# JGCRI/xanthos

Hardware: AMD Instinct MI355X
Metric: cell-months/sec (pm_abcd_mrtm, 67,420 cells) (higher is better)
Workload: dtype f64

## Files before the change

### include/xanthos_hip.h

```cpp
#ifndef XANTHOS_HIP_H
#define XANTHOS_HIP_H

#include <stddef.h>
#include <stdint.h>

#ifdef __cplusplus
extern "C" {
#endif

#define XH_OK 0
#define XH_ERR_ARG 1
#define XH_ERR_HIP 2
#define XH_ERR_LIMIT 3
#define XH_ERR_DEVICE 4

#define XH_MAX_LCS 32

typedef struct xh_ctx xh_ctx;
typedef struct xh_route_plan xh_route_plan;

int xh_abi_version(void);
int xh_device_count(int *n);
int xh_ctx_create(int device, xh_ctx **out);
void xh_ctx_destroy(xh_ctx *ctx);
// ... 39 lines not shown
int xh_timing_reset(xh_ctx *ctx);
int xh_mark_begin(xh_ctx *ctx, const char *name);
int xh_mark_end(xh_ctx *ctx);
int xh_timing_enable(xh_ctx *ctx, int on);
int xh_timing_get(xh_ctx *ctx, const char *name, double *total_ms, int64_t *launches);

typedef struct xh_pm_tables {
    int32_t nlcs;
    const double *cL, *beta, *rslimit, *Tminopen, *Tminclose, *VPDclose, *VPDopen, *RBLmin, *RBLmax, *rc,
        *emiss;
    const double *alpha, *lai, *laimin, *laimax;
} xh_pm_tables;

int xh_pm_pet(xh_ctx *ctx, const xh_pm_tables *h_tab,
              int64_t ncell, int32_t nmonths,
              int32_t start_year,
              int32_t n_lc_years, const int32_t *h_lc_years,
              int32_t water_idx, int32_t snow_idx,
              const double *d_tas, const double *d_tmin, const double *d_rhs, const double *d_wind,
              const double *d_rsds, const double *d_rlds,
              const double *d_tairprev,
              const double *d_lct,
              const double *d_elev,
              double *d_pet);

int xh_abcd(xh_ctx *ctx, int64_t ncell, int32_t nmonths, int32_t spinup, int32_t n_groups,
            const int32_t *h_basin_index, const int32_t *h_par_index, int64_t npar_rows, const double *d_pars,
            const double *d_pet, const double *d_precip, const double *d_tmin,
            double *d_aet, double *d_q, double *d_sav,
            double *d_sm0, double *d_gw0);

int xh_hargreaves_pet(xh_ctx *ctx, int64_t ncell, int32_t nmonths,
                      const double *d_temp, const double *d_dtr,
                      const double *d_lat_rad,
                      const double *h_solar_dec, const double *h_dr, const double *h_ndays,
                      double *d_pet);

int xh_hs_pet(xh_ctx *ctx, int64_t ncell, int32_t nmonths,
              const double *d_tas, const double *d_tmax, const double *d_tmin,
              const double *d_lat_deg,
              const double *h_ndays,
              double *d_pet);

#define XH_DAYLIGHT_REFERENCE 0
#define XH_DAYLIGHT_MONTHLY 1
int xh_thornthwaite_pet(xh_ctx *ctx, int64_t ncell, int32_t nmonths, int32_t start_year, int32_t daylight_mode,
                        const double *d_tas,
                        const double *d_lat_rad,
                        double *d_pet,
                        double *d_daylight);

int xh_gwam(xh_ctx *ctx, int64_t ncell, int32_t nmonths, int32_t spinup, int32_t precip_col_spinup,
            int32_t precip_col_sim, double indexing,
            const double *d_pet, const double *d_precip,
            const double *d_sm_max, const double *d_sm0,
            double *d_aet, double *d_q, double *d_sav,
            double *d_sm_end);

int xh_route_plan_create(xh_ctx *ctx, int64_t ncell, const int64_t *h_indptr, const int32_t *h_indices,
                         const int8_t *h_sign, xh_route_plan **out);
void xh_route_plan_destroy(xh_route_plan *plan);
int xh_route_plan_info(const xh_route_plan *plan, int64_t info[16]);

int xh_route_plan_prepare(xh_ctx *ctx, xh_route_plan *plan, const double *h_flow_dist, const double *h_velocity, double dt);

int xh_route_plan_stats(xh_route_plan *plan, int64_t max_words, uint64_t *h_words, int64_t *n_words);

int xh_mrtm_downstream(int64_t ncell, int32_t nrow, int32_t ncol, const int64_t *h_id, const int32_t *h_ilon,
                       const int32_t *h_ilat, const double *h_flowdir, int64_t *h_dsid);
int xh_mrtm_upstream(int64_t ncell, int32_t nrow, int32_t ncol, const int64_t *h_id, const int32_t *h_ilon,
                     const int32_t *h_ilat, const int64_t *h_dsid, int64_t *h_upid);
int xh_mrtm_um_csr(int64_t ncell, const int64_t *h_upid, int64_t *h_indptr, int32_t *h_indices, int8_t *h_sign);

#define XH_ROUTE_DEFAULT 0
#define XH_ROUTE_FORCE_FALLBACK 1
#define XH_ROUTE_ATOMIC 2
#define XH_ROUTE_NO_DATAFLOW 4
#define XH_ROUTE_NO_SKEW 8
#define XH_ROUTE_TEST_FAULT 16
#define XH_ROUTE_VALIDATE 32
#define XH_ROUTE_REASSOC 128
#define XH_ROUTE_EXACT 256
int xh_route_plan_rsum_info(const xh_route_plan *plan, int64_t info[8]);
int xh_route_series(xh_ctx *ctx, xh_route_plan *plan, int32_t nmonths, int32_t spinup_months,
                    const int32_t *h_ndays, double dt,
                    const double *d_flow_dist, const double *d_velocity, const double *d_area,
                    const double *d_runoff, const double *d_S0,
                    double *d_chstorage, double *d_avgchflow, double *d_S_end, double *d_F_end, int32_t flags);

typedef struct xh_fused_args {
    int64_t ncell;
    int32_t nmonths, start_year;
    const xh_pm_tables *pm;
    int32_t n_lc_years;
    const int32_t *h_lc_years;
    int32_t water_idx, snow_idx;
    const double *d_tas, *d_tmin, *d_rhs, *d_wind, *d_rsds, *d_rlds, *d_tairprev, *d_lct, *d_elev;
    int32_t abcd_spinup, n_groups;
    const int32_t *h_basin_index, *h_par_index;
    int64_t npar_rows;
    const double *d_pars, *d_precip, *d_abcd_tmin;
    xh_route_plan *plan;
    int32_t routing_spinup;
    const int32_t *h_ndays;
    double dt;
    const double *d_flow_dist, *d_velocity, *d_area, *d_S0;
    int32_t route_flags;
    double *d_pet, *d_aet, *d_q, *d_sav, *d_chstorage, *d_avgchflow;
    int32_t block_months;
    int32_t mode;
} xh_fused_args;
int xh_run_fused(xh_ctx *ctx, const xh_fused_args *args);

int xh_calib_objective(xh_ctx *ctx, int64_t ncell_b, int32_t nmonths, int32_t spinup, int32_t nmembers,
                       int32_t npar, const double *h_pars, const double *d_pet_t, const double *d_precip_t,
                       const double *d_tmin_t, const double *d_area, const double *h_obs, double *h_ed,
                       double *h_series);

int xh_agg_time(xh_ctx *ctx, int64_t ncell, int32_t ncols, int32_t group, int32_t mode, const double *d_scale,
                const double *d_in, double *d_out);
int xh_agg_spatial(xh_ctx *ctx, int64_t ncell, int32_t ncols, int32_t n_groups, const int32_t *h_group,
                   const double *d_in, double *d_out);
int xh_nan_to_num(xh_ctx *ctx, double *d_arr, int64_t n);

int xh_drought_thresholds(xh_ctx *ctx, int64_t ncell, int32_t nmonths, int32_t month0, int32_t nyear, int32_t nper,
                          int32_t k_prev, int32_t k_next, double gamma, const double *d_hydro, double *d_thresh);
int xh_drought_stats(xh_ctx *ctx, int64_t ncell, int32_t nmonths, int32_t nthresh, const double *d_hydro,
                     const double *d_thresh, double *d_severity, double *d_intensity, double *d_duration);

int xh_hpot_qmax(xh_ctx *ctx, int64_t ncell, int32_t nmonths, int32_t k_prev, int32_t k_next, double gamma,
                 const double *d_q, double *d_qmax);
int xh_hpot_energy(xh_ctx *ctx, int64_t ncell, int32_t nmonths, int32_t nyears, const int32_t *d_year_of_month,
                   double c_ef_sww, double c_hours, double c_twh, double c_ej, const double *d_q, const double *d_qmax,
                   const double *d_elev, double *d_E);
int xh_hpot_region(xh_ctx *ctx, int32_t ngroups, int32_t nyears, const int64_t *d_indptr, const int64_t *d_cells,
                   const double *d_E, double *d_R);

int xh_hact_inflow(xh_ctx *ctx, int64_t ncell, int32_t nmonths, int32_t ndams, int32_t month0, const int64_t *d_dam_cell,
                   const double *d_catch, const double *d_assumed, double cumecs_to_mm3, const double *d_q, double *d_inflow,
                   double *d_env, int32_t *d_bad);
int xh_hact_sim(xh_ctx *ctx, int32_t nmonths, int32_t ndams, int32_t nyears, int32_t month0, const int32_t *d_year_of_month,
                double sww, double secs_in_month, const double *d_inflow, const double *d_env, const double *d_rc,
                const double *d_par, double *d_power, double *d_annual, int32_t *d_bad_month);

int xh_diag_cell_total(xh_ctx *ctx, int64_t ncell, int32_t ncols, const double *d_in, double div1, const double *d_scale,
                       double div2, double *d_out, int64_t out_stride);
int xh_diag_group_sum(xh_ctx *ctx, int64_t ncell, int32_t k, int32_t ngroups, const int32_t *h_group, const double *d_vals,
                      double *d_sums, int64_t *d_counts);

#define XH_ENS_MEAN 1u
#define XH_ENS_STD 2u
#define XH_ENS_MIN 4u
#define XH_ENS_MAX 8u
int xh_ens_stats(xh_ctx *ctx, int64_t n, int32_t nmembers, const double *const *h_d_members, uint32_t stat_mask,
                 int32_t nq, const double *h_q, double *const *h_d_out);

int xh_basin_kge(xh_ctx *ctx, int64_t ncell, int32_t nmonths, int32_t nbasins, const int64_t *d_start,
                 const int32_t *d_cells, const double *d_q, const double *d_area, const double *d_obs, double *d_series,
                 double *d_ed);

int xh_gauge_skill(xh_ctx *ctx, int64_t ncell, int32_t nmonths, int32_t ngauge, const int32_t *d_gauge_cell,
                   const double *d_flow, const double *d_obs, double *d_series, double *d_metrics);

#define XH_STD_INDEX_GAMMA 0
#define XH_STD_INDEX_EMPIRICAL 1
int xh_std_index(xh_ctx *ctx, int64_t ncell, int32_t nmonths, int32_t nscale, const int32_t *h_scale, int32_t ref_month0,
// ... 131 lines not shown
```

### xanthos_amd/_hip.py

```python
import contextlib
import ctypes
import os
import threading
from ctypes import POINTER, Structure, byref, c_char_p, c_double, c_int, c_int8, c_int32, c_int64, c_size_t, \
    c_uint64, c_void_p

import numpy as np

_HERE = os.path.dirname(os.path.abspath(__file__))
LIB_PATH = os.environ.get('XH_LIBRARY') or os.path.join(_HERE, 'libxanthos_hip.so')

XH_ROUTE_DEFAULT, XH_ROUTE_FORCE_FALLBACK, XH_ROUTE_ATOMIC, XH_ROUTE_NO_DATAFLOW, XH_ROUTE_NO_SKEW = 0, 1, 2, 4, 8
XH_ROUTE_TEST_FAULT, XH_ROUTE_VALIDATE = 16, 32
XH_ROUTE_REASSOC, XH_ROUTE_EXACT = 128, 256
XH_ROUTE_NO_PLAIN = 0x4000
XH_DAYLIGHT_REFERENCE, XH_DAYLIGHT_MONTHLY = 0, 1
XH_ERR_ARG, XH_ERR_HIP, XH_ERR_LIMIT, XH_ERR_DEVICE = 1, 2, 3, 4
XH_SRC_F32_LE, XH_SRC_F32_BE, XH_SRC_F64_BE = 1, 2, 3
NARROW_KINDS = {np.dtype('<f4'): (XH_SRC_F32_LE, 'f32'), np.dtype('>f4'): (XH_SRC_F32_BE, 'f32be'),
                np.dtype('>f8'): (XH_SRC_F64_BE, 'f64be')}
STD_INDEX_DIST = {'gamma': 0, 'empirical': 1}
STD_INDEX_DIST2 = dict(STD_INDEX_DIST, loglogistic=2)
ENS_STAT_BITS = {'mean': 1, 'std': 2, 'min': 4, 'max': 8}

# ... 27 lines not shown


class CalibFlowDesc(Structure):
    _fields_ = [('routing_spinup', c_int32), ('dt', c_double)] + [(n, c_void_p) for n in (
        'h_ndays', 'h_closure_ptr', 'h_row_ptr', 'h_cols', 'h_sign', 'h_basin_col', 'h_outlet_rank', 'h_tauinv', 'h_area',
        'h_s0')]


def flow_desc(tables):
    t = tables
    return CalibFlowDesc(int(t.routing_spinup), float(t.dt), *[_host_ptr(a) for a in (
        t.ndays, t.closure_ptr, t.row_ptr, t.cols, t.sign, t.basin_col, t.outlet_rank, t.tauinv, t.area, t.s0)])


class CalibGaugeDesc(Structure):
    _fields_ = [('routing_spinup', c_int32), ('dt', c_double)] + [(n, c_void_p) for n in (
        'h_ndays', 'h_closure_ptr', 'h_row_ptr', 'h_cols', 'h_sign', 'h_basin_col', 'h_tauinv', 'h_area', 'h_s0',
        'h_gauge_ptr', 'h_gauge_row', 'h_gauge_weight')]


def gauge_desc(tables):
    t = tables
    return CalibGaugeDesc(int(t.routing_spinup), float(t.dt), *[_host_ptr(a) for a in (
        t.ndays, t.closure_ptr, t.row_ptr, t.cols, t.sign, t.basin_col, t.tauinv, t.area, t.s0, t.gauge_ptr, t.gauge_row,
        t.gauge_weight)])


class CalibVelocityDesc(Structure):
    _fields_ = [('h_velocity', c_void_p), ('h_length', c_void_p)]


def velocity_desc(tables):
    return CalibVelocityDesc(_host_ptr(tables.velocity), _host_ptr(tables.length))


_P = c_void_p
SIGNATURES = {
    'xh_abi_version': (c_int, []),
    'xh_device_count': (c_int, [POINTER(c_int)]),
    'xh_ctx_create': (c_int, [c_int, POINTER(c_void_p)]),
    'xh_ctx_destroy': (None, [_P]),
    'xh_last_error': (c_char_p, [_P]),
    'xh_device_name': (c_int, [_P, ctypes.c_char_p, c_size_t]),
    'xh_malloc': (c_int, [_P, c_size_t, POINTER(c_void_p)]),
    'xh_free': (c_int, [_P, _P]),
    'xh_mem_info': (c_int, [_P, POINTER(c_size_t), POINTER(c_size_t)]),
    'xh_memcpy_h2d': (c_int, [_P, _P, _P, c_size_t]),
    'xh_memcpy_d2h': (c_int, [_P, _P, _P, c_size_t]),
    'xh_memcpy_d2d': (c_int, [_P, _P, _P, c_size_t]),
    'xh_host_alloc': (c_int, [_P, c_size_t, POINTER(c_void_p)]),
    'xh_host_free': (c_int, [_P, _P]),
    'xh_memcpy_h2d_async': (c_int, [_P, _P, _P, c_size_t]),
    'xh_memcpy_d2h_async': (c_int, [_P, _P, _P, c_size_t]),
    'xh_upload_file': (c_int, [_P, _P, c_char_p, ctypes.c_uint64, c_size_t, c_int]),
    'xh_download_file': (c_int, [_P, _P, c_char_p, ctypes.c_uint64, c_size_t, c_int]),
    'xh_download_files': (c_int, [_P, c_int, POINTER(c_void_p), POINTER(c_char_p), POINTER(ctypes.c_uint64), POINTER(c_size_t)]),
    'xh_csv_format': (c_int, [_P, _P, c_int64, c_int64, c_int64, _P, c_size_t, _P]),
    'xh_csv_write': (c_int, [_P, _P, c_int64, c_int64, c_int64, c_char_p, ctypes.c_uint64, c_size_t, POINTER(ctypes.c_uint64)]),
    'xh_csv_write_many': (c_int, [_P, c_int, POINTER(c_void_p), POINTER(c_int64), POINTER(c_int64), POINTER(c_int64),
                                  POINTER(c_char_p), POINTER(ctypes.c_uint64), c_size_t, POINTER(ctypes.c_uint64)]),
    'xh_pack_f32_be': (c_int, [_P, _P, c_int64, _P]),
    'xh_grid_pack_f32_be': (c_int, [_P, _P, c_int64, c_int64, _P, c_int64, ctypes.c_uint32, _P]),
    'xh_widen': (c_int, [_P, _P, c_int, c_int64, _P]),
    'xh_memset': (c_int, [_P, _P, c_int, c_size_t]),
    'xh_sync': (c_int, [_P]),
    'xh_gather_rows': (c_int, [_P, _P, _P, c_int64, c_int64, _P]),
    'xh_scatter_rows': (c_int, [_P, _P, _P, c_int64, c_int64, _P]),
    'xh_transpose': (c_int, [_P, _P, c_int64, c_int64, _P]),
    'xh_timing_reset': (c_int, [_P]),
    'xh_timing_enable': (c_int, [_P, c_int]),
    'xh_timing_get': (c_int, [_P, c_char_p, POINTER(c_double), POINTER(c_int64)]),
    'xh_pm_pet': (c_int, [_P, POINTER(PmTables), c_int64, c_int32, c_int32, c_int32, _P, c_int32, c_int32,
                          _P, _P, _P, _P, _P, _P, _P, _P, _P, _P]),
    'xh_abcd': (c_int, [_P, c_int64, c_int32, c_int32, c_int32, _P, _P, c_int64, _P, _P, _P, _P, _P, _P, _P, _P, _P]),
    'xh_hargreaves_pet': (c_int, [_P, c_int64, c_int32, _P, _P, _P, _P, _P, _P, _P]),
    'xh_gwam': (c_int, [_P, c_int64, c_int32, c_int32, c_int32, c_int32, c_double, _P, _P, _P, _P, _P, _P, _P, _P]),
    'xh_hs_pet': (c_int, [_P, c_int64, c_int32, _P, _P, _P, _P, _P, _P]),
    'xh_thornthwaite_pet': (c_int, [_P, c_int64, c_int32, c_int32, c_int32, _P, _P, _P, _P]),
    'xh_route_plan_create': (c_int, [_P, c_int64, _P, _P, _P, POINTER(c_void_p)]),
    'xh_route_plan_destroy': (None, [_P]),
    'xh_route_plan_info': (c_int, [_P, POINTER(c_int64)]),
    'xh_route_plan_stats': (c_int, [_P, c_int64, _P, POINTER(c_int64)]),
    'xh_route_plan_rsum_info': (c_int, [_P, POINTER(c_int64)]),
    'xh_route_plan_prepare': (c_int, [_P, _P, _P, _P, c_double]),
    'xh_mrtm_downstream': (c_int, [c_int64, c_int32, c_int32, _P, _P, _P, _P, _P]),
    'xh_mrtm_upstream': (c_int, [c_int64, c_int32, c_int32, _P, _P, _P, _P, _P]),
    'xh_mrtm_um_csr': (c_int, [c_int64, _P, _P, _P, _P]),
    'xh_route_series': (c_int, [_P, _P, c_int32, c_int32, _P, c_double, _P, _P, _P, _P, _P, _P, _P, _P, _P, c_int32]),
    'xh_run_fused': (c_int, [_P, POINTER(FusedArgs)]),
    'xh_calib_objective': (c_int, [_P, c_int64, c_int32, c_int32, c_int32, c_int32, _P, _P, _P, _P, _P, _P, _P, _P]),
    'xh_calib_objective_multi': (c_int, [_P, c_int32, _P, c_int32, c_int32, c_int32, c_int32, _P, _P, _P, _P, _P, _P, _P, _P]),
    'xh_calib_de_create': (c_int, [_P, c_int32, _P, _P, c_int32, c_int32, c_int32, c_int32, _P, _P, _P, _P, _P, _P, _P,
                                   c_uint64, POINTER(c_void_p)]),
    'xh_calib_flow_objective_multi': (c_int, [_P, c_int32, _P, c_int32, c_int32, c_int32, c_int32, _P, _P, _P, _P,
                                              POINTER(CalibFlowDesc), _P, _P, _P]),
    'xh_calib_de_create_flow': (c_int, [_P, c_int32, _P, _P, c_int32, c_int32, c_int32, c_int32, _P, _P, _P,
                                        POINTER(CalibFlowDesc), _P, _P, _P, c_uint64, POINTER(c_void_p)]),
    'xh_calib_gauge_objective_multi': (c_int, [_P, c_int32, _P, c_int32, c_int32, c_int32, c_int32, _P, _P, _P, _P,
                                               POINTER(CalibGaugeDesc), _P, _P, _P, _P]),
    'xh_calib_de_create_gauge': (c_int, [_P, c_int32, _P, _P, c_int32, c_int32, c_int32, c_int32, _P, _P, _P,
                                         POINTER(CalibGaugeDesc), _P, _P, _P, c_uint64, POINTER(c_void_p)]),
    'xh_calib_flow_velocity_objective_multi': (c_int, [_P, c_int32, _P, c_int32, c_int32, c_int32, c_int32, _P, _P, _P, _P,
                                                       POINTER(CalibFlowDesc), POINTER(CalibVelocityDesc), _P, _P, _P]),
    'xh_calib_gauge_velocity_objective_multi': (c_int, [_P, c_int32, _P, c_int32, c_int32, c_int32, c_int32, _P, _P, _P, _P,
                                                        POINTER(CalibGaugeDesc), POINTER(CalibVelocityDesc), _P, _P, _P,
                                                        _P]),
    'xh_calib_de_create_flow_velocity': (c_int, [_P, c_int32, _P, _P, c_int32, c_int32, c_int32, c_int32, _P, _P, _P,
                                                 POINTER(CalibFlowDesc), POINTER(CalibVelocityDesc), _P, _P, _P, c_uint64,
                                                 POINTER(c_void_p)]),
    'xh_calib_de_create_gauge_velocity': (c_int, [_P, c_int32, _P, _P, c_int32, c_int32, c_int32, c_int32, _P, _P, _P,
                                                  POINTER(CalibGaugeDesc), POINTER(CalibVelocityDesc), _P, _P, _P, c_uint64,
                                                  POINTER(c_void_p)]),
    'xh_calib_de_destroy': (None, [_P]),
    'xh_calib_de_init': (c_int, [_P]),
    'xh_calib_de_step': (c_int, [_P, c_int32, c_double, c_double, c_double, c_double, c_double, POINTER(c_int32)]),
    'xh_calib_de_result': (c_int, [_P, _P, _P, _P, _P, _P]),
    'xh_calib_de_state': (c_int, [_P, c_int32, _P, _P]),
    'xh_calib_de_set_state': (c_int, [_P, _P, _P, c_int32]),
    'xh_comm_unique_id': (c_int, [ctypes.c_char_p, c_size_t]),
    'xh_comm_create': (c_int, [_P, c_int32, c_int32, ctypes.c_char_p, c_size_t, POINTER(c_void_p)]),
    'xh_comm_destroy': (None, [_P]),
    'xh_comm_info': (c_int, [_P, POINTER(c_int64)]),
    'xh_comm_gather_rows': (c_int, [_P, _P, c_int32, c_int32, _P, c_int64, _P, _P, _P]),
    'xh_comm_gather_rows_side': (c_int, [_P, _P, c_int32, c_int32, _P, c_int64, _P, _P, _P]),
    'xh_comm_join': (c_int, [_P]),
    'xh_mark_begin': (c_int, [_P, c_char_p]),
    'xh_mark_end': (c_int, [_P]),
    'xh_agg_time': (c_int, [_P, c_int64, c_int32, c_int32, c_int32, _P, _P, _P]),
    'xh_agg_spatial': (c_int, [_P, c_int64, c_int32, c_int32, _P, _P, _P]),
    'xh_nan_to_num': (c_int, [_P, _P, c_int64]),
    'xh_drought_thresholds': (c_int, [_P, c_int64, c_int32, c_int32, c_int32, c_int32, c_int32, c_int32, c_double, _P, _P]),
    'xh_drought_stats': (c_int, [_P, c_int64, c_int32, c_int32, _P, _P, _P, _P, _P]),
    'xh_hpot_qmax': (c_int, [_P, c_int64, c_int32, c_int32, c_int32, c_double, _P, _P]),
    'xh_hpot_energy': (c_int, [_P, c_int64, c_int32, c_int32, _P, c_double, c_double, c_double, c_double, _P, _P, _P, _P]),
    'xh_hpot_region': (c_int, [_P, c_int32, c_int32, _P, _P, _P, _P]),
    'xh_hact_inflow': (c_int, [_P, c_int64, c_int32, c_int32, c_int32, _P, _P, _P, c_double, _P, _P, _P, _P]),
    'xh_hact_sim': (c_int, [_P, c_int32, c_int32, c_int32, c_int32, _P, c_double, c_double, _P, _P, _P, _P, _P, _P, _P]),
    'xh_diag_cell_total': (c_int, [_P, c_int64, c_int32, _P, c_double, _P, c_double, _P, c_int64]),
    'xh_diag_group_sum': (c_int, [_P, c_int64, c_int32, c_int32, _P, _P, _P, _P]),
    'xh_ens_stats': (c_int, [_P, c_int64, c_int32, POINTER(c_void_p), ctypes.c_uint32, c_int32, _P, POINTER(c_void_p)]),
    'xh_basin_kge': (c_int, [_P, c_int64, c_int32, c_int32, _P, _P, _P, _P, _P, _P, _P]),
    'xh_gauge_skill': (c_int, [_P, c_int64, c_int32, c_int32, _P, _P, _P, _P, _P]),
    'xh_std_index': (c_int, [_P, c_int64, c_int32, c_int32, POINTER(c_int32), c_int32, c_int32, c_int32, c_double, _P,
                            POINTER(c_void_p), POINTER(c_void_p), POINTER(c_void_p)]),
    'xh_std_index2': (c_int, [_P, c_int64, c_int32, c_int32, POINTER(c_int32), c_int32, c_int32, c_int32, c_double, _P, _P,
                             POINTER(c_void_p), POINTER(c_void_p), POINTER(c_void_p)]),
    'xh_synth_forcing': (c_int, [_P, c_uint64, c_double, c_int64, c_int32, _P, _P, _P, _P, _P, _P, _P, _P, _P, _P]),
}

_lib = None


ABI_VERSION = 7


def lib():
    global _lib
    if _lib is None:
        if not os.path.isfile(LIB_PATH):
            raise HipUnavailable(
                '{} not found: build it with `python -c "import __graft_entry__ as g; g.build()"` or '
                '`make -C xanthos_amd/csrc` (hipcc --offload-arch=gfx950). There is no CPU fallback.'.format(LIB_PATH))
        try:
            handle = ctypes.CDLL(LIB_PATH)
        except OSError as exc:
            raise HipUnavailable('cannot load {}: {}'.format(LIB_PATH, exc))
        for name, (res, args) in SIGNATURES.items():
            try:
                fn = getattr(handle, name)
            except AttributeError:
                raise HipUnavailable('{} lacks {}: it was built from older sources; rebuild it (make -C xanthos_amd/csrc)'
                                     .format(LIB_PATH, name))
            fn.restype = res
            fn.argtypes = args
        if handle.xh_abi_version() != ABI_VERSION:
            raise HipUnavailable('{} has ABI version {}, this package binds version {}: rebuild it (make -C xanthos_amd/csrc)'
                                 .format(LIB_PATH, handle.xh_abi_version(), ABI_VERSION))
        _lib = handle
    return _lib


def _host_ptr(arr):
    return arr.ctypes.data_as(c_void_p)


def as_f64(a):
    return np.ascontiguousarray(a, dtype=np.float64)


class DeviceArray:

    def __init__(self, ctx, shape, dtype=np.float64):
        self.ctx = ctx
        self.shape = tuple(int(s) for s in (shape if isinstance(shape, (tuple, list)) else (shape,)))
        self.dtype = np.dtype(dtype)
        self.nbytes = int(np.prod(self.shape, dtype=np.int64)) * self.dtype.itemsize
        p = c_void_p()
        ctx._check(lib().xh_malloc(ctx.handle, self.nbytes, byref(p)))
        self.ptr = p.value
        ctx._live.add(self)

    @property
    def size(self):
        return int(np.prod(self.shape, dtype=np.int64))

    def upload(self, host):
        host = np.ascontiguousarray(host, dtype=self.dtype)
        if host.nbytes != self.nbytes:
            raise ValueError('size mismatch: host {} vs device {}'.format(host.shape, self.shape))
        self.ctx._check(lib().xh_memcpy_h2d(self.ctx.handle, self.ptr, _host_ptr(host), self.nbytes))
        return self

    def download(self, out=None):
        if out is None:
            out = np.empty(self.shape, dtype=self.dtype)
        if out.nbytes != self.nbytes or not out.flags.c_contiguous:
            raise ValueError('bad output buffer')
        self.ctx._check(lib().xh_memcpy_d2h(self.ctx.handle, _host_ptr(out), self.ptr, self.nbytes))
        return out

    def zero(self):
        self.ctx._check(lib().xh_memset(self.ctx.handle, self.ptr, 0, self.nbytes))
        return self

    def free(self):
        if self.ptr is not None and self.ctx.handle is not None:
            lib().xh_free(self.ctx.handle, self.ptr)
            self.ctx._live.discard(self)
        self.ptr = None

    def __del__(self):
        try:
            self.free()
        except Exception:
            pass


def _dptr(x):
    if x is None:
        return None
    if isinstance(x, DeviceArray):
        return x.ptr
    return int(x)


class Context:

    def __init__(self, device=0):
        L = lib()
        h = c_void_p()
        rc = L.xh_ctx_create(int(device), byref(h))
        if rc != 0:
            msg = L.xh_last_error(None)
# ... 441 lines not shown
    def diag_group_sum(self, ncell, k, ngroups, group_index, vals, sums, counts):
        gi = np.ascontiguousarray(group_index, dtype=np.int32)
        self._check(lib().xh_diag_group_sum(self.handle, ncell, k, ngroups, _host_ptr(gi), _dptr(vals), _dptr(sums),
                                            _dptr(counts)))

    def ens_stats(self, n, members, stats=(), quantiles=(), out=None):
        unknown = [s for s in stats if s not in ENS_STAT_BITS]
        if unknown:
            raise ValueError('unknown ensemble statistic {}'.format(unknown))
        mask = 0
        for s in stats:
            mask |= ENS_STAT_BITS[s]
        q = np.ascontiguousarray(quantiles, dtype=np.float64).reshape(-1)
        nout = bin(mask).count('1') + q.size
        if out is None or len(out) != nout:
            raise ValueError('{} statistics need {} output arrays'.format(nout, nout))
        nmem = len(members)
        p_mem = (c_void_p * max(nmem, 1))(*[_dptr(m) for m in members])
        p_out = (c_void_p * max(nout, 1))(*[_dptr(o) for o in out])
        self._check(lib().xh_ens_stats(self.handle, int(n), nmem, p_mem, mask, q.size, _host_ptr(q) if q.size else None,
                                       p_out))

    def basin_kge(self, ncell, nmonths, nbasins, start, cells, q, area, obs, ed, series=None):
        self._check(lib().xh_basin_kge(self.handle, int(ncell), int(nmonths), int(nbasins), _dptr(start), _dptr(cells),
                                       _dptr(q), _dptr(area), _dptr(obs), _dptr(series), _dptr(ed)))

    def gauge_skill(self, ncell, nmonths, ngauge, gauge_cell, flow, obs, metrics, series=None):
        self._check(lib().xh_gauge_skill(self.handle, int(ncell), int(nmonths), int(ngauge), _dptr(gauge_cell), _dptr(flow),
                                         _dptr(obs), _dptr(series), _dptr(metrics)))

    def std_index(self, ncell, nmonths, scales, ref_month0, ref_nyear, dist, max_shape, x, index, par_in=None, par_out=None,
                  minus=None):
        if dist not in STD_INDEX_DIST2:
            raise ValueError("unknown distribution '{}' (gamma, empirical or loglogistic)".format(dist))
        k = np.ascontiguousarray(scales, dtype=np.int32).reshape(-1)
        for name, arrs in (('index', index), ('par_in', par_in), ('par_out', par_out)):
            if arrs is not None and len(arrs) != k.size:
                raise ValueError('{} scales need {} {} arrays, not {}'.format(k.size, k.size, name, len(arrs)))

        def table(arrs):
            return None if arrs is None else (c_void_p * max(k.size, 1))(*[_dptr(a) for a in arrs])
        self._check(lib().xh_std_index2(self.handle, int(ncell), int(nmonths), int(k.size), k.ctypes.data_as(POINTER(c_int32)),
                                        int(ref_month0), int(ref_nyear), STD_INDEX_DIST2[dist], float(max_shape), _dptr(x),
                                        _dptr(minus), table(par_in), table(par_out), table(index)))

    def synth_forcing(self, seed, ncell, nmonths, lat, out, nan_frac=0.001, cell_ids=None):
        g = lambda k: _dptr(out.get(k))
        self._check(lib().xh_synth_forcing(self.handle, int(seed), float(nan_frac), ncell, nmonths, _dptr(lat),
                                           _dptr(cell_ids), g('tas'), g('tmin'), g('rhs'), g('wind'), g('rsds'),
                                           g('rlds'), g('precip'), g('abcd_tmin')))


class RoutePlan:

    def __init__(self, ctx, indptr, indices, sign):
        self.ctx = ctx
        ip = np.ascontiguousarray(indptr, dtype=np.int64)
        ix = np.ascontiguousarray(indices, dtype=np.int32)
        sg = np.ascontiguousarray(sign, dtype=np.int8)
        self.ncell = ip.size - 1
        h = c_void_p()
        ctx._check(lib().xh_route_plan_create(ctx.handle, self.ncell, _host_ptr(ip), _host_ptr(ix), _host_ptr(sg),
                                              byref(h)))
        self.handle = h.value

    def info(self):
        arr = (c_int64 * 16)()
        self.ctx._check(lib().xh_route_plan_info(self.handle, arr))
        keys = ('networks', 'largest_network', 'units', 'fallback_cells', 'largest_unit', 'slots', 'single_downstream',
                'flow_units', 'flow_edges', 'flow_depth', 'flow_cells', 'flow_max_imports', 'skew_max_lag',
                'last_tree_kernel', 'reroutes', 'validated')
        return dict(zip(keys, list(arr)))

    def prepare(self, flow_dist, velocity, dt):
        L = np.ascontiguousarray(flow_dist, dtype=np.float64)
        v = np.ascontiguousarray(velocity, dtype=np.float64)
        if L.size != self.ncell or v.size != self.ncell:
            raise ValueError('flow_dist / velocity must have one value per cell')
        self.ctx._check(lib().xh_route_plan_prepare(self.ctx.handle, self.handle, _host_ptr(L), _host_ptr(v), float(dt)))

    def rsum_info(self):
        arr = (c_int64 * 8)()
        self.ctx._check(lib().xh_route_plan_rsum_info(self.handle, arr))
        return dict(zip(('units', 'folded', 'fold_disabled', 'prepared_folded', 'pair_cells', 'prepared_pair_cells', 'guard_trips',
                         'pair_units'), list(arr)))

    def stats(self):
        n = c_int64(0)
        self.ctx._check(lib().xh_route_plan_stats(self.handle, 0, None, byref(n)))
        if n.value == 0:
            return None
        out = np.empty(n.value, dtype=np.uint64)
        self.ctx._check(lib().xh_route_plan_stats(self.handle, n.value, _host_ptr(out), byref(n)))
        return out.reshape(-1, 6)

    def close(self):
        if self.handle is not None and self.ctx.handle is not None:
            lib().xh_route_plan_destroy(self.handle)
        self.handle = None

    def __del__(self):
        try:
            self.close()
        except Exception:
            pass


def comm_unique_id():
    buf = ctypes.create_string_buffer(128)
    _check_host(lib().xh_comm_unique_id(buf, 128))
    return buf.raw


class Comm:

    def __init__(self, ctx, nranks, rank, unique_id):
        self.ctx, self.nranks, self.rank = ctx, int(nranks), int(rank)
        h = c_void_p()
        import sys
        sys.stdout.flush()
        saved = os.dup(1)
        try:
            os.dup2(2, 1)
            rc = lib().xh_comm_create(ctx.handle, self.nranks, self.rank, unique_id, len(unique_id), byref(h))
            ctypes.CDLL(None).fflush(None)
        finally:
            os.dup2(saved, 1)
            os.close(saved)
        ctx._check(rc)
        self.handle = h.value

    def info(self):
        arr = (c_int64 * 4)()
        self.ctx._check(lib().xh_comm_info(self.handle, arr))
        return dict(zip(('ranks', 'rank', 'sends', 'recvs'), list(arr)))

    def gather_rows(self, local, counts, ncols, perm=None, out=None, root=0, side=False):
        nvar = len(local)
        cn = np.ascontiguousarray(counts, dtype=np.int64)
        p_local = (c_void_p * nvar)(*[_dptr(x) for x in local])
        p_out = None if out is None else (c_void_p * nvar)(*[_dptr(x) for x in out])
        fn = lib().xh_comm_gather_rows_side if side else lib().xh_comm_gather_rows
        self.ctx._check(fn(self.ctx.handle, self.handle, int(root), nvar, p_local, int(ncols), _host_ptr(cn), _dptr(perm),
                           p_out))

    def close(self):
        if self.handle is not None:
            lib().xh_comm_destroy(self.handle)
        self.handle = None

    def __del__(self):
        try:
            self.close()
        except Exception:
            pass


class CalibDE:

    def __init__(self, ctx, ncells, nmonths, spinup, nmembers, bounds, pet_t, precip_t, tmin_t, area, obs, seed=0,
                 keys=None, flow=None, velocity=False):
        self.ctx = ctx
        nc = np.ascontiguousarray(ncells, dtype=np.int64)
        self.nb, self.n, self.d = int(nc.size), int(nmembers), len(bounds)
        obs = as_f64(obs)
        gauge_form = flow is not None and hasattr(flow, 'gauge_ptr')
        if obs.shape != ((int(flow.gauge_ptr[-1]) if gauge_form else self.nb), nmonths):
            raise ValueError('obs must be [ngauge, nmonths]' if gauge_form else 'obs must be [nbasins, nmonths]')
# ... 150 lines not shown
```

### xanthos_amd/csrc/xh_flow_plan.cpp

```cpp
#include "xh_flow_plan.h"

#include <unistd.h>

#include <algorithm>
#include <cstdio>
#include <numeric>
#include <thread>
#include <type_traits>
#include <utility>

using xh_flow::Tree;
using xh_flow::tree_analyse;

namespace {

constexpr int W_MAX = 9;
constexpr int LANES = 64;
constexpr int G_MAX = 16;
constexpr int NPAIR = 2 * LANES + 1;
constexpr int SK_P = 4;
constexpr unsigned SK_ZERO = 2u * LANES * 16u;

}

// ... 815 lines not shown
        if (t.export_edge[slot_of[pc]] != ed) return fail("export_edge of the producer");
        if (t.edge_cons_unit[ed] != cu) return fail("edge_cons_unit");
        if (pu == cu && t.piece_of_cell[pc] == t.piece_of_cell[cc]) return fail("stream inside a piece");
        if (t.unit_depth[pu] >= t.unit_depth[cu] && !(t.unit_depth[pu] == 0 && t.unit_depth[cu] == 0 && false))
            return fail("stream from depth " + std::to_string(t.unit_depth[pu]) + " to depth " + std::to_string(t.unit_depth[cu]));
        imp[cu]++;
        exp[pu]++;
    }
    for (int u = 0; u < t.n_units; ++u) {
        if (imp[u] > G_MAX || exp[u] > G_MAX) return fail("more than 16 imports / outlets in unit " + std::to_string(u));
        int g = 0;
        for (int k = 0; k < LANES; ++k)
            if (t.ghost_edge[(int64_t)u * LANES + k] >= 0) {
                if (k != g) return fail("ghost entries are not packed from 0");
                ++g;
            }
        if (g != imp[u]) return fail("ghost count");
        if (t.unit_lmax[u] & 15) return fail("unit lag not a multiple of 16");
    }
    auto expand = [&](int u, unsigned off, std::vector<int> &terms, int depth, auto &&self) -> bool {
        if (off == SK_ZERO) return true;
        const int e = (int)(off / 16u);
        if (off % 16u) return false;
        if (e >= LANES) {
            const int ed = t.ghost_edge[(int64_t)u * LANES + (e - LANES)];
            if (ed < 0) return false;
            terms.push_back(t.edge_prod_cell[ed]);
            return true;
        }
        const int64_t s = (int64_t)u * LANES + e;
        const int c = t.cell_of_slot[s];
        if (c < 0 || depth > LANES) return false;
        if ((t.unit_p[u] & 0x100) && t.eprev[s] != SK_ZERO && !self(u, t.eprev[s], terms, depth + 1, self)) return false;
        terms.push_back(c);
        return true;
    };
    auto lag_of = [&](int u, unsigned off) {
        const int e = (int)(off / 16u);
        return e >= LANES ? t.ghost_lag[(int64_t)u * LANES + (e - LANES)] : t.lag[(int64_t)u * LANES + e];
    };
    std::vector<int> terms, want;
    for (int c = 0; c < n; ++c) {
        if (!handled[c]) continue;
        const int s = slot_of[c], u = s / LANES;
        if (t.lag[s] < 0 || t.lag[s] > t.unit_lmax[u] || (t.lag[s] & 1)) return fail("lag of cell " + std::to_string(c));
        const bool chained = (t.unit_p[u] & 0x100) != 0;
        if (chained && t.eprev[s] != SK_ZERO && t.lag[s] - lag_of(u, t.eprev[s]) != 2) return fail("chain lag");
        if (!chained && t.eprev[s] != SK_ZERO) return fail("eprev in a unit that is not chained");
        const int upre = t.unit_p[u] & 15, upost = (t.unit_p[u] >> 4) & 15;
        for (int side = 0; side < 2; ++side) {
            terms.clear();
            want.clear();
            bool past = false;
            for (int64_t j = indptr[c]; j < indptr[c + 1]; ++j) {
                if (indices[j] == c) past = true;
                else if (past == (side == 1)) want.push_back(indices[j]);
            }
            for (int w = 0; w < SK_P; ++w) {
                const unsigned off = t.ent2[(size_t)(side * SK_P + w) * ts + s];
                if (off == SK_ZERO) continue;
                if (w >= (side ? upost : upre)) return fail("row longer than the unit's shape at cell " + std::to_string(c));
                if (t.lag[s] - lag_of(u, off) != 2) return fail("a gathered value is not two iterations old at cell " + std::to_string(c));
                if (side == 1) {
                    const int e = (int)(off / 16u);
                    if (e < LANES && chained && t.eprev[(int64_t)u * LANES + e] != SK_ZERO) return fail("chain member read from behind a diagonal");
                }
                if (!expand(u, off, terms, 0, expand)) return fail("bad table entry at cell " + std::to_string(c));
            }
            if (terms != want) return fail("row of cell " + std::to_string(c) + " does not expand to its CSR row");
        }
        if (chained && t.eprev[s] != SK_ZERO && t.ds[c] < 0) return fail("chain member without a downstream cell");
    }
    for (int ed = 0; ed < t.n_edges; ++ed) {
        const int cu = slot_of[t.edge_cons_cell[ed]] / LANES;
        bool found = false;
        for (int k = 0; k < LANES && !found; ++k)
            found = t.ghost_edge[(int64_t)cu * LANES + k] == ed && t.ghost_prod[(int64_t)cu * LANES + k] == t.edge_prod_cell[ed];
        if (!found) return fail("ghost_prod of stream " + std::to_string(ed));
    }
    return "";
}

namespace {
constexpr unsigned long long TABLES_MAGIC = 0x3472546c66485806ull;

template <class T>
bool put_vec(FILE *f, const std::vector<T> &v) {
    const unsigned long long n = v.size();
    return fwrite(&n, sizeof(n), 1, f) == 1 && (n == 0 || fwrite(v.data(), sizeof(T), n, f) == n);
}
template <class T>
bool get_vec(FILE *f, std::vector<T> &v) {
    unsigned long long n = 0;
    if (fread(&n, sizeof(n), 1, f) != 1 || n > (1ull << 31)) return false;
    {
        const long here = ftell(f);
        if (here < 0 || fseek(f, 0, SEEK_END) != 0) return false;
        const long end = ftell(f);
        if (end < here || fseek(f, here, SEEK_SET) != 0 || n > (unsigned long long)(end - here) / sizeof(T)) return false;
    }
    v.resize((size_t)n);
    return n == 0 || fread(v.data(), sizeof(T), n, f) == n;
}
template <class F>
bool tables_io(FILE *f, FlowTables &t, bool write, F &&vec) {
    int head[13] = {t.n_units, t.n_edges, t.depth, t.n_cells, t.max_imports, t.max_exports, t.skew_ok ? 1 : 0,
                    t.skew_lmax, t.skew_span, t.rsum ? 1 : 0, t.n_folded, t.n_special, t.n_pair_units};
    if (write ? fwrite(head, sizeof(head), 1, f) != 1 : fread(head, sizeof(head), 1, f) != 1) return false;
    if (!write) {
        t.n_units = head[0], t.n_edges = head[1], t.depth = head[2], t.n_cells = head[3], t.max_imports = head[4];
        t.max_exports = head[5], t.skew_ok = head[6] != 0, t.skew_lmax = head[7];
        t.skew_span = head[8], t.rsum = head[9] != 0, t.n_folded = head[10], t.n_special = head[11], t.n_pair_units = head[12];
    }
    return vec(t.cell_of_slot) && vec(t.export_edge) && vec(t.ghost_edge) && vec(t.edge_cons_unit) && vec(t.unit_terms) &&
           vec(t.ent) && vec(t.lag) && vec(t.ghost_lag) && vec(t.unit_p) && vec(t.unit_lmax) && vec(t.unit_glmax) &&
           vec(t.unit_order) && vec(t.ent2) && vec(t.eprev) && vec(t.edge_prod_cell) && vec(t.edge_cons_cell) &&
           vec(t.unit_depth) && vec(t.piece_of_cell) && vec(t.unit_of_cell) && vec(t.height_of_cell) && vec(t.ds) &&
           vec(t.lane_flags) && vec(t.ghost_prod) && vec(t.fold_of_slot);
}
}

bool flow_tables_save(const FlowTables &t, const char *path) {
    const std::string tmp = std::string(path) + ".tmp." + std::to_string((long long)getpid());
    FILE *f = fopen(tmp.c_str(), "wb");
    if (!f) return false;
    FlowTables &m = const_cast<FlowTables &>(t);
    bool ok = fwrite(&TABLES_MAGIC, sizeof(TABLES_MAGIC), 1, f) == 1 &&
              tables_io(f, m, true, [&](auto &v) { return put_vec(f, v); });
    ok = fclose(f) == 0 && ok;
    if (ok) ok = rename(tmp.c_str(), path) == 0;
    if (!ok) (void)remove(tmp.c_str());
    return ok;
}

bool flow_tables_load(const char *path, FlowTables &t) {
    FILE *f = fopen(path, "rb");
    if (!f) return false;
    unsigned long long magic = 0;
    t = FlowTables();
    bool ok = false;
    try {
        ok = fread(&magic, sizeof(magic), 1, f) == 1 && magic == TABLES_MAGIC &&
             tables_io(f, t, false, [&](auto &v) { return get_vec(f, v); }) && fgetc(f) == EOF;
    } catch (...) {
        ok = false;
    }
    fclose(f);
    if (!ok) t = FlowTables();
    return ok;
}
```

### xanthos_amd/csrc/xh_flow_plan.h

```cpp
#pragma once
#include <cstdint>
#include <string>
#include <vector>

struct FlowPlanOptions {
    int simds = 0;
    int piece_cap = 0;
    bool chain = true;
    bool cut_rule = true;
    int tlimit = 5;
    bool balance_lds = false;
    int lane_trials = 0;
    bool debug = false;
    const unsigned char *foldable = nullptr;
    const unsigned char *capable = nullptr;
    int halo = 8;
    int pair_imports = 8;
};

struct FlowTables {
    int n_units = 0, n_edges = 0, depth = 0, n_cells = 0, max_imports = 0, max_exports = 0;
    bool skew_ok = false;
    int skew_lmax = 0;
    int skew_span = 1;
    bool rsum = false;
    std::vector<int> cell_of_slot, export_edge, ghost_edge, edge_cons_unit, unit_terms;
    std::vector<unsigned> ent;
    std::vector<int> lag, ghost_lag, unit_p, unit_lmax, unit_glmax, unit_order;
    std::vector<unsigned> ent2, eprev;
    std::vector<int> edge_prod_cell, edge_cons_cell, unit_depth, piece_of_cell, unit_of_cell, height_of_cell, ds;
    std::vector<unsigned char> lane_flags;
    std::vector<int> ghost_prod;
    std::vector<int> fold_of_slot;
    int n_folded = 0;
    int n_special = -1;
    int n_pair_units = 0;
};

namespace xh_flow {
struct Tree {
    int n = 0;
    const int64_t *indptr = nullptr;
    const int32_t *indices = nullptr;
    const int8_t *sign = nullptr;
    std::vector<int> ds, nchild, child_ptr, child, cell_pre, cell_post;
    std::vector<char> ok;
};
void tree_analyse(int n, const int64_t *indptr, const int32_t *indices, const int8_t *sign, const int *comp, int ncomp,
                  Tree &t);
}

int flow_tables_build(int n, const int64_t *indptr, const int32_t *indices, const int8_t *sign, const int *comp,
                      int ncomp, const FlowPlanOptions &opt, std::vector<char> &handled, FlowTables &out,
                      std::string &err);

std::string flow_tables_check(int n, const int64_t *indptr, const int32_t *indices, const int8_t *sign,
                              const std::vector<char> &handled, const FlowTables &t);

int flow_tables_build_rsum(int n, const int64_t *indptr, const int32_t *indices, const int8_t *sign, const int *comp,
                           int ncomp, const FlowPlanOptions &opt, std::vector<char> &handled, FlowTables &out,
                           std::string &err);
std::string flow_tables_check_rsum(int n, const int64_t *indptr, const int32_t *indices, const int8_t *sign,
                                   const std::vector<char> &handled, const FlowTables &t);
int flow_rsum_planner_version();

bool flow_tables_save(const FlowTables &t, const char *path);
bool flow_tables_load(const char *path, FlowTables &t);
```

### xanthos_amd/csrc/xh_flow_rsum.cpp

```cpp
#include <algorithm>
#include <cstdio>
#include <numeric>
#include <string>
#include <thread>

#include "xh_flow_plan.h"

using xh_flow::Tree;
using xh_flow::tree_analyse;

namespace {

constexpr int LANES = 64;
constexpr int G_MAX = 16;
constexpr int W_MAX = 9;
constexpr int SK_P = 4;
constexpr unsigned SK_ZERO = 2u * LANES * 16u;
constexpr int H_MAX = 88;

struct RPart {
    std::vector<int> queue, piece, roots, psize, pimp, pdepth;
    std::vector<int> e_prod, e_cons, e_kind;
    std::vector<int> unit_of_piece, unit_cells, unit_imp, unit_out, unit_depth;
    std::vector<char> unit_cheap, unit_special, special, mayfire;
// ... 239 lines not shown
                put_piece(p, u);
                taken[p] = 1;
            }
        }
        std::vector<int> by_size;
        for (int p : fre)
            if (!taken[p]) by_size.push_back(p);
        std::stable_sort(by_size.begin(), by_size.end(), [&](int x, int y) { return P.psize[x] > P.psize[y]; });
        {
            std::vector<std::vector<int>> bucket(LANES + 1);
            for (int u = 0; u < (int)P.unit_cells.size(); ++u)
                if (!P.unit_cheap[u] && !P.unit_special[u]) bucket[LANES - P.unit_cells[u]].push_back(u);
            for (int p : by_size) {
                const int sz = P.psize[p];
                int u = -1;
                if (special[roots[p]]) {
                    for (int b = 0; b < (int)P.unit_cells.size() && u < 0; ++b)
                        if (P.unit_special[b] && P.unit_cells[b] + sz <= LANES) u = b;
                    if (u < 0) {
                        u = new_unit(0, false);
                        P.unit_special[u] = 1;
                    }
                    put_piece(p, u);
                    continue;
                }
                for (int f = sz; f <= LANES && u < 0; ++f)
                    for (size_t i = bucket[f].size(); i-- > 0;) {
                        const int b = bucket[f][i];
                        if (has_fold[p] && (P.unit_imp[b] > 0 || P.unit_out[b] > 0)) continue;
                        u = b;
                        bucket[f].erase(bucket[f].begin() + (long)i);
                        break;
                    }
                if (u < 0) u = new_unit(0, false);
                put_piece(p, u);
                bucket[LANES - P.unit_cells[u]].push_back(u);
            }
        }
        P.nunit = (int)P.unit_cells.size();
        P.n_cheap = cheap;
        int npair = 0;
        for (char c : P.unit_special) npair += c ? 1 : 0;
        const int simds_left = opt.simds - (opt.simds >= 64 ? std::min(3 * npair, opt.simds / 4) : 0);
        need = opt.simds > 0 ? std::max(P.nunit - simds_left, 0) : 0;
        if (need <= cheap || !cheap_units) break;
        cheap = need + (round > 0 ? 2 : 0);
    }
    return need;
    };
    int need = pack(false);
    for (int pass = 0; pass < 4 && need > 0 && opt.foldable; ++pass) {
        std::vector<int> gain(npiece, 0);
        for (int c : queue) {
            const int q = P.piece[c];
            if (q < 0 || special[c] || fold_leaf[c] >= 0 || P.pimp[q] != 0) continue;
            for (int k = child_ptr[c]; k < child_ptr[c + 1]; ++k)
                if (opt.foldable[child[k]] && t.nchild[child[k]] == 0 && P.piece[child[k]] == q) {
                    gain[q]++;
                    break;
                }
        }
        std::vector<int> order;
        for (int p = 0; p < npiece; ++p)
            if (gain[p] > 0) order.push_back(p);
        std::stable_sort(order.begin(), order.end(), [&](int x, int y) { return gain[x] > gain[y]; });
        const int want = (need + 1) * LANES + LANES / 2;
        std::vector<char> chosen(npiece, 0);
        int got = 0;
        for (int p : order) {
            if (got >= want) break;
            chosen[p] = 1;
            got += gain[p];
        }
        if (got == 0) break;
        fold_pieces([&](int p) { return chosen[p] != 0; });
        mark_folds();
        need = pack(false);
    }
    if (need > 0) pack(true);
}

}

int flow_rsum_planner_version() { return 8; }

int flow_tables_build_rsum(int n, const int64_t *indptr, const int32_t *indices, const int8_t *sign, const int *comp,
                           int ncomp, const FlowPlanOptions &opt, std::vector<char> &handled, FlowTables &out,
                           std::string &err) {
    out = FlowTables();
    out.rsum = true;
    handled.assign(n, 0);
    if (n == 0) return 0;
    Tree t;
    tree_analyse(n, indptr, indices, sign, comp, ncomp, t);
    const std::vector<int> &ds = t.ds;

    RPart P;
    std::vector<int> fold_leaf;
    {
        static const int caps[] = {LANES, 56, 48, 44, 40, 36, 32, 28, 24};
        constexpr int NCAP = (int)(sizeof(caps) / sizeof(caps[0]));
        std::vector<RPart> cand(opt.piece_cap > 0 ? 1 : NCAP);
        std::vector<std::vector<int>> cand_fold(cand.size());
        if (cand.size() == 1 || n < 4096) {
            for (size_t k = 0; k < cand.size(); ++k)
                rsum_partition(t, opt, opt.piece_cap > 0 ? std::min(opt.piece_cap, LANES) : caps[k], cand[k], cand_fold[k]);
        } else {
            std::vector<std::thread> pool;
            for (size_t k = 0; k < cand.size(); ++k) pool.emplace_back([&, k] { rsum_partition(t, opt, caps[k], cand[k], cand_fold[k]); });
            for (auto &th : pool) th.join();
        }
        bool have = false;
        long best_score = 0;
        for (size_t k = 0; k < cand.size(); ++k) {
            RPart &Q = cand[k];
            int indep = 0;
            for (int u = 0; u < Q.nunit; ++u) indep += (Q.unit_imp[u] == 0 && Q.unit_out[u] == 0) ? 1 : 0;
            int npair = 0;
            for (char c : Q.unit_special) npair += c ? 1 : 0;
            const int extra = opt.simds > 0 ? std::max(Q.nunit - (opt.simds - (opt.simds >= 64 ? std::min(3 * npair, opt.simds / 4) : 0)), 0) : 0;
            std::vector<char> ufold(Q.nunit, 0);
            for (int c = 0; c < n; ++c)
                if (cand_fold[k][c] >= 0) ufold[Q.unit_of_piece[Q.piece[c]]] = 1;
            int fold_streams = 0;
            for (int u = 0; u < Q.nunit; ++u) fold_streams += (ufold[u] && (Q.unit_imp[u] > 0 || Q.unit_out[u] > 0)) ? 1 : 0;
            const long score = 1000000L * std::max(2 * extra - indep, 0) + 20000L * fold_streams + 1000L * Q.nunit + Q.nedge / 8;
            if (opt.debug)
                fprintf(stderr, "flow plan (reassociated): piece capacity %d -> %d units, %d streams, %d units without streams, depth %d\n",
                        opt.piece_cap > 0 ? opt.piece_cap : caps[k], Q.nunit, Q.nedge, indep, Q.maxdepth + 1);
            if (!have || score < best_score) {
                std::swap(P, Q);
                std::swap(fold_leaf, cand_fold[k]);
                best_score = score;
                have = true;
            }
        }
    }
    const std::vector<int> &piece = P.piece, &roots = P.roots, &unit_of_piece = P.unit_of_piece;
    const int nunit = P.nunit, nedge = P.nedge;
    if (nunit == 0) return 0;
    const int64_t ts = (int64_t)nunit * LANES;

    out.cell_of_slot.assign(ts, -1);
    out.export_edge.assign(ts, -1);
    out.ghost_edge.assign(ts, -1);
    out.ghost_prod.assign(ts, 0);
    out.edge_cons_unit.assign(nedge, 0);
    std::vector<int> slot_of_cell(n, -1), fill(nunit, 0), gfill(nunit, 0), edge_ghost(nedge, 0);
    for (int c = 0; c < n; ++c)
        if (piece[c] >= 0) {
            const int u = unit_of_piece[piece[c]];
            const int s = fill[u]++;
            if (s >= LANES) {
                err = "flow plan (reassociated): a unit holds more than 64 cells";
                return -1;
            }
            out.cell_of_slot[(int64_t)u * LANES + s] = c;
            slot_of_cell[c] = s;
            handled[c] = 1;
        }
    for (int c = 0; c < n; ++c)
        if (fold_leaf[c] >= 0) {
            if (piece[c] < 0) {
                err = "flow plan (reassociated): a folded leaf lost its carrier";
                return -1;
            }
            if (out.fold_of_slot.empty()) out.fold_of_slot.assign(ts, -1);
// ... 26 lines not shown
            if (piece[t.child[k]] >= 0 && piece[t.child[k]] == piece[c]) kids.push_back(t.child[k]);
        std::stable_sort(kids.begin(), kids.end(), [&](int x, int y) { return th[x] < th[y]; });
        const int p = (int)kids.size();
        int h = edge_in0[c] >= 0 ? (p > 0 ? p + 1 : 1) : 0;
        for (int i = 0; i < p; ++i) h = std::max(h, 1 + (p - 1 - i) + th[kids[i]]);
        th[c] = h;
        for (int i = 0; i < p; ++i) r_src[kids[i]] = i > 0 ? kids[i - 1] : (edge_in0[c] >= 0 ? -2 - edge_in0[c] : -1);
        a_src[c] = p > 0 ? kids[p - 1] : (edge_in0[c] >= 0 ? -2 - edge_in0[c] : -1);
        for (int i = 0; i < p; ++i) hgt[kids[i]] = p - 1 - i;
    }
    std::vector<int> unit_h(nunit, 0), edge_reader_h(nedge, 0);
    for (size_t qi = P.queue.size(); qi-- > 0;) {
        const int c = P.queue[qi];
        if (piece[c] < 0) continue;
        const bool root = roots[piece[c]] == c;
        if (root) {
            hgt[c] = 0;
            if (edge_in1[c] >= 0) r_src[c] = -2 - edge_in1[c];
        } else {
            hgt[c] = hgt[ds[c]] + 1 + hgt[c];
        }
        int &uh = unit_h[unit_of_piece[piece[c]]];
        uh = std::max(uh, hgt[c]);
    }
    for (int c = 0; c < n; ++c) {
        if (piece[c] < 0) continue;
        for (int src : {a_src[c], r_src[c]})
            if (src <= -2) {
                const int ed = -2 - src;
                edge_reader_h[ed] = hgt[c];
                int &uh = unit_h[out.edge_cons_unit[ed]];
                uh = std::max(uh, hgt[c] + 1);
            }
    }

    out.lag.assign(ts, 0);
    out.ghost_lag.assign(ts, 0);
    out.unit_p.assign(nunit, 0x400);
    out.unit_lmax.assign(nunit, 0);
    out.unit_glmax.assign(nunit, 0);
    out.ent2.assign((size_t)2 * SK_P * ts, SK_ZERO);
    out.eprev.assign(ts, SK_ZERO);
    out.ent.assign((size_t)W_MAX * ts, SK_ZERO);
    out.unit_terms.assign(nunit, 1);
    for (int u = 0; u < nunit; ++u) out.unit_lmax[u] = (2 * unit_h[u] + 15) & ~15;
    auto entry_of = [&](int src, int u) -> unsigned {
        if (src == -1) return SK_ZERO;
        if (src <= -2) return (unsigned)(LANES + edge_ghost[-2 - src]) * 16u;
        (void)u;
        return (unsigned)slot_of_cell[src] * 16u;
    };
    for (int c = 0; c < n; ++c) {
        if (piece[c] < 0) continue;
        const int u = unit_of_piece[piece[c]];
        const int64_t slot = (int64_t)u * LANES + slot_of_cell[c];
        out.lag[slot] = out.unit_lmax[u] - 2 * hgt[c];
        out.ent2[(size_t)slot] = entry_of(a_src[c], u);
        out.eprev[slot] = entry_of(r_src[c], u);
        if (a_src[c] != -1) out.unit_p[u] |= 1;
        if (r_src[c] != -1) out.unit_p[u] |= 2;
        if (fold_leaf[c] >= 0) out.unit_p[u] |= 4;
    }
    out.n_special = P.n_special;
    out.n_pair_units = 0;
    if (P.n_special >= 0)
        for (int u = 0; u < nunit; ++u) {
            out.unit_p[u] |= P.unit_special[u] ? 24 : 8;
            out.n_pair_units += P.unit_special[u] ? 1 : 0;
        }
    for (int ed = 0; ed < nedge; ++ed) {
        const int u = out.edge_cons_unit[ed];
        const int gl = out.unit_lmax[u] - 2 * (edge_reader_h[ed] + 1);
        out.ghost_lag[(int64_t)u * LANES + edge_ghost[ed]] = gl;
        out.unit_glmax[u] = std::max(out.unit_glmax[u], gl);
    }
    out.lane_flags.assign(ts, 0);
    if (P.n_special >= 0)
        for (int64_t sl = 0; sl < ts; ++sl) {
            const int c = out.cell_of_slot[sl];
            if (c < 0) continue;
            out.lane_flags[sl] = (unsigned char)((P.mayfire[c] ? 1 : 0) | ((P.special[c] && ds[c] >= 0 && !P.special[ds[c]]) ? 2 : 0));
        }

    std::vector<int> unit_exp(nunit, 0);
    for (int ed = 0; ed < nedge; ++ed) unit_exp[unit_of_piece[piece[P.e_prod[ed]]]]++;
    {
        std::vector<int> cost(nunit);
        for (int u = 0; u < nunit; ++u)
            cost[u] = 100 + 25 * ((out.unit_p[u] & 1) + ((out.unit_p[u] >> 1) & 1)) + (P.unit_imp[u] > 0 ? 15 : 0) + (unit_exp[u] > 0 ? 15 : 0);
        auto coupled = [&](int u) { return P.unit_imp[u] > 0 || unit_exp[u] > 0; };
        out.unit_order.resize(nunit);
        std::iota(out.unit_order.begin(), out.unit_order.end(), 0);
        auto pairu = [&](int u) { return P.n_special >= 0 && P.unit_special[u]; };
        std::stable_sort(out.unit_order.begin(), out.unit_order.end(), [&](int x, int y) {
            if (pairu(x) != pairu(y)) return !pairu(x);
            if (coupled(x) != coupled(y)) return !coupled(x);
            if (cost[x] != cost[y]) return cost[x] < cost[y];
            return P.unit_cells[x] < P.unit_cells[y];
        });
    }

    out.skew_ok = true;
    out.skew_lmax = *std::max_element(out.unit_lmax.begin(), out.unit_lmax.end());
    {
        int span = 1;
        for (int ed = 0; ed < nedge; ++ed) span = std::max(span, P.pdepth[piece[P.e_cons[ed]]] - P.pdepth[piece[P.e_prod[ed]]]);
        out.skew_span = span;
    }
    out.n_units = nunit;
    out.n_edges = nedge;
    out.depth = P.maxdepth + 1;
    out.n_cells = (int)std::count(handled.begin(), handled.end(), (char)1);
    out.max_imports = *std::max_element(P.unit_imp.begin(), P.unit_imp.end());
    out.max_exports = *std::max_element(unit_exp.begin(), unit_exp.end());
    out.edge_prod_cell = P.e_prod;
    out.edge_cons_cell = P.e_cons;
    out.unit_depth = P.unit_depth;
    out.piece_of_cell = piece;
    out.unit_of_cell.assign(n, -1);
    for (int c = 0; c < n; ++c)
        if (piece[c] >= 0) out.unit_of_cell[c] = unit_of_piece[piece[c]];
    out.height_of_cell = hgt;
    out.ds = ds;

    if (opt.debug) {
        std::vector<int> hs(4, 0), hl(14, 0), hi(6, 0);
        int indep = 0;
        for (int u = 0; u < nunit; ++u) {
            hs[out.unit_p[u] & 3]++;
            hl[std::min(out.unit_lmax[u] / 16, 13)]++;
            hi[P.unit_imp[u] == 0 ? 0 : P.unit_imp[u] <= 2 ? 1 : P.unit_imp[u] <= 4 ? 2 : P.unit_imp[u] <= 8 ? 3 : 4]++;
            indep += (P.unit_imp[u] == 0 && unit_exp[u] == 0) ? 1 : 0;
        }
        fprintf(stderr, "flow plan (reassociated): %d units (%d without streams, %d kept cheap), %d pieces, %d streams, depth %d, %lld of %lld lanes used\n",
                nunit, indep, P.n_cheap, (int)roots.size(), nedge, P.maxdepth + 1, (long long)out.n_cells, (long long)ts);
        {
            int nfu = 0, nfi = 0;
            for (int u = 0; u < nunit; ++u) {
                nfu += (out.unit_p[u] & 4) ? 1 : 0;
                nfi += ((out.unit_p[u] & 4) && (P.unit_imp[u] > 0 || unit_exp[u] > 0)) ? 1 : 0;
            }
            fprintf(stderr, "  folded leaves: %d, in %d units (of them with streams: %d)\n", out.n_folded, nfu, nfi);
        }
        {
            int nsu = 0;
            for (int u = 0; u < nunit; ++u) nsu += (out.unit_p[u] & 16) ? 1 : 0;
            int nx = 0;
            for (int c = 0; c < n; ++c) nx += (P.n_special >= 0 && P.mayfire[c]) ? 1 : 0;
            int quiet = 0;
            for (int u = 0; u < nunit && P.n_special >= 0; ++u) {
                bool any = (out.unit_p[u] & 16) != 0;
                for (int k = 0; k < LANES && !any; ++k) any = (out.lane_flags[(int64_t)u * LANES + k] & 1) != 0;
                quiet += any ? 0 : 1;
            }
            for (int u = 0; u < nunit && P.n_special >= 0; ++u)
                if (out.unit_p[u] & 16)
                    fprintf(stderr, "  pair unit %d: %d cells, %d imports, %d outlets, depth %d, lmax %d\n", u, P.unit_cells[u], P.unit_imp[u], unit_exp[u],
                            P.unit_depth[u], out.unit_lmax[u]);
            fprintf(stderr, "  single-sum plan: %s, %d cells may fire, %d of them in pair form in %d units; %d single units hold no cell that may fire\n",
                    P.n_special >= 0 ? "yes" : "no", nx, std::max(P.n_special, 0), nsu, quiet);
        }
        fprintf(stderr, "  units by reads (none, A, R, A+R): %d %d %d %d\n  units by lmax/16 (0..13+):", hs[0], hs[1], hs[2], hs[3]);
        for (int k = 0; k < 14; ++k) fprintf(stderr, " %d", hl[k]);
        fprintf(stderr, "\n  units by imports (0, <=2, <=4, <=8, more): %d %d %d %d %d\n  longest stream jump: %d levels\n", hi[0], hi[1],
                hi[2], hi[3], hi[4], out.skew_span);
    }
    return 0;
}

std::string flow_tables_check_rsum(int n, const int64_t *indptr, const int32_t *indices, const int8_t *sign,
                                   const std::vector<char> &handled, const FlowTables &t) {
    if (!t.rsum) return "not a reassociated plan";
    if (t.n_units == 0) {
        for (int c = 0; c < n; ++c)
            if (handled[c]) return "handled cell without units";
        return "";
    }
    const int64_t ts = (int64_t)t.n_units * LANES;
    if ((int64_t)t.cell_of_slot.size() != ts || (int64_t)t.lag.size() != ts || (int64_t)t.eprev.size() != ts ||
        (int64_t)t.ent2.size() != 2 * SK_P * ts || (int)t.unit_p.size() != t.n_units || (int64_t)t.ghost_edge.size() != ts ||
        (int64_t)t.ghost_lag.size() != ts || (int64_t)t.export_edge.size() != ts || (int)t.unit_lmax.size() != t.n_units ||
        (int)t.unit_order.size() != t.n_units || (int)t.edge_cons_unit.size() != t.n_edges ||
        (int)t.edge_prod_cell.size() != t.n_edges || (int)t.edge_cons_cell.size() != t.n_edges || (int)t.ds.size() != n ||
        (int)t.unit_depth.size() != t.n_units)
        return "table sizes";
    std::vector<int> slot_of(n, -1);
    for (int64_t s = 0; s < ts; ++s) {
        const int c = t.cell_of_slot[s];
        if (c < 0) continue;
        if (c >= n || !handled[c]) return "slot holds a cell that is not handled";
        if (slot_of[c] >= 0) return "cell " + std::to_string(c) + " sits in two slots";
        slot_of[c] = (int)s;
    }
    std::vector<int> carrier(n, -1);
    if (!t.fold_of_slot.empty()) {
        if ((int64_t)t.fold_of_slot.size() != ts) return "fold table size";
        for (int64_t s = 0; s < ts; ++s) {
            const int l = t.fold_of_slot[s];
            if (l < 0) continue;
            const int c = t.cell_of_slot[s];
            if (c < 0 || l >= n || !handled[l] || slot_of[l] >= 0 || carrier[l] >= 0) return "folded leaf " + std::to_string(l);
            if (t.ds[l] != c) return "folded leaf " + std::to_string(l) + " is not carried by its downstream cell";
            if (indptr[l + 1] - indptr[l] != 1) return "folded cell " + std::to_string(l) + " is not a leaf";
            if (!(t.unit_p[s / LANES] & 4)) return "unit shape lacks the fold flag";
            carrier[l] = c;
        }
    }
    for (int c = 0; c < n; ++c)
        if (handled[c] && slot_of[c] < 0 && carrier[c] < 0) return "handled cell " + std::to_string(c) + " has no slot";
    {
        std::vector<char> seen(t.n_units, 0);
        for (int u : t.unit_order) {
            if (u < 0 || u >= t.n_units || seen[u]) return "claim list is not a permutation of the units";
            seen[u] = 1;
        }
    }
    std::vector<int> imp(t.n_units, 0), exp(t.n_units, 0);
    for (int ed = 0; ed < t.n_edges; ++ed) {
        const int pc = t.edge_prod_cell[ed], cc = t.edge_cons_cell[ed];
        if (pc < 0 || pc >= n || cc < 0 || cc >= n || slot_of[pc] < 0 || slot_of[cc] < 0) return "stream between cells that are not routed";
        if (t.ds[pc] != cc && !(t.ds[pc] >= 0 && t.ds[pc] == t.ds[cc])) return "stream follows neither a flow edge nor a sibling link";
        const int pu = slot_of[pc] / LANES, cu = slot_of[cc] / LANES;
        if (t.export_edge[slot_of[pc]] != ed) return "export_edge of the producer";
        if (t.edge_cons_unit[ed] != cu) return "edge_cons_unit";
        if (t.unit_depth[pu] >= t.unit_depth[cu]) return "stream from depth " + std::to_string(t.unit_depth[pu]) + " to depth " + std::to_string(t.unit_depth[cu]);
        imp[cu]++;
        exp[pu]++;
    }
    for (int u = 0; u < t.n_units; ++u) {
        if (imp[u] > G_MAX || exp[u] > G_MAX) return "more than 16 imports / outlets in unit " + std::to_string(u);
        int g = 0;
        for (int k = 0; k < LANES; ++k)
            if (t.ghost_edge[(int64_t)u * LANES + k] >= 0) {
                if (k != g) return "ghost entries are not packed from 0";
                if (t.ghost_edge[(int64_t)u * LANES + k] >= t.n_edges || t.edge_cons_unit[t.ghost_edge[(int64_t)u * LANES + k]] != u)
                    return "ghost entry of a stream that does not end in the unit";
                if (t.ghost_prod[(int64_t)u * LANES + k] != t.edge_prod_cell[t.ghost_edge[(int64_t)u * LANES + k]]) return "ghost_prod";
                ++g;
            }
        if (g != imp[u]) return "ghost count";
        if (t.unit_lmax[u] & 15) return "unit lag not a multiple of 16";
        if ((t.unit_p[u] & ~31) != 0x400) return "shape word of unit " + std::to_string(u);
        if (t.n_special >= 0 ? !(t.unit_p[u] & 8) : (t.unit_p[u] & 24) != 0) return "single-sum flags of unit " + std::to_string(u);
    }
    std::vector<int> readers_lane(ts, 0), readers_ghost(t.n_edges, 0);
    auto expand = [&](int u, unsigned off, std::vector<int> &terms, int depth, auto &&self) -> bool {
        if (off == SK_ZERO) return true;
        if (off % 16u) return false;
        const int e = (int)(off / 16u);
        if (e >= 2 * LANES || depth > 4 * LANES + t.n_edges) return false;
        if (e >= LANES) {
            const int ed = t.ghost_edge[(int64_t)u * LANES + (e - LANES)];
            if (ed < 0) return false;
            const int ps = slot_of[t.edge_prod_cell[ed]];
            return self(ps / LANES, (unsigned)(ps % LANES) * 16u, terms, depth + 1, self);
        }
        const int64_t s = (int64_t)u * LANES + e;
        const int c = t.cell_of_slot[s];
        if (c < 0) return false;
        if (!self(u, t.eprev[s], terms, depth + 1, self)) return false;
        terms.push_back(c);
        return true;
    };
    auto lag_of = [&](int u, unsigned off) {
        const int e = (int)(off / 16u);
        return e >= LANES ? t.ghost_lag[(int64_t)u * LANES + (e - LANES)] : t.lag[(int64_t)u * LANES + e];
    };
    auto note_reader = [&](int u, unsigned off) {
        if (off == SK_ZERO) return;
        const int e = (int)(off / 16u);
        if (e >= LANES) readers_ghost[t.ghost_edge[(int64_t)u * LANES + (e - LANES)]]++;
        else readers_lane[(int64_t)u * LANES + e]++;
    };
    std::vector<int> terms, want;
    for (int c = 0; c < n; ++c) {
        if (!handled[c] || slot_of[c] < 0) continue;
        const int s = slot_of[c], u = s / LANES;
        if (t.lag[s] < 0 || t.lag[s] > t.unit_lmax[u] || (t.lag[s] & 1)) return "lag of cell " + std::to_string(c);
        const unsigned a = t.ent2[(size_t)s], r = t.eprev[s];
        for (int w = 1; w < 2 * SK_P; ++w)
            if (t.ent2[(size_t)w * ts + s] != SK_ZERO) return "a reassociated plan reads one inflow entry per cell";
        for (unsigned off : {a, r}) {
            if (off == SK_ZERO) continue;
            if (off % 16u || off / 16u >= 2u * LANES) return "bad table entry at cell " + std::to_string(c);
            const int e = (int)(off / 16u);
            if (e >= LANES ? t.ghost_edge[(int64_t)u * LANES + (e - LANES)] < 0 : t.cell_of_slot[(int64_t)u * LANES + e] < 0)
                return "cell " + std::to_string(c) + " reads an empty entry";
            if (t.lag[s] - lag_of(u, off) != 2) return "a value read is not two iterations old at cell " + std::to_string(c);
            note_reader(u, off);
        }
        if (a != SK_ZERO && !(t.unit_p[u] & 1)) return "unit shape lacks the inflow read";
        if (r != SK_ZERO && !(t.unit_p[u] & 2)) return "unit shape lacks the chain read";
        terms.clear();
        if (!expand(u, a, terms, 0, expand)) return "bad chain at cell " + std::to_string(c);
        if (t.n_special >= 0) {
            if ((int64_t)t.lane_flags.size() != ts) return "lane flags";
            const bool pair_u = (t.unit_p[u] & 16) != 0;
            if (pair_u && !(t.lane_flags[s] & 1)) return "cell " + std::to_string(c) + " of a pair unit is not one that may fire";
            if (pair_u && !t.fold_of_slot.empty() && t.fold_of_slot[s] >= 0) return "folded leaf in a pair unit";
            int nx = 0;
            bool seen_pair = false, order_ok = true;
            for (int x : terms) {
                const bool xp = (t.unit_p[slot_of[x] / LANES] & 16) != 0;
                if ((t.lane_flags[slot_of[x]] & 1)) {
                    ++nx;
                    if ((t.lane_flags[s] & 1) && !xp) return "neighbour " + std::to_string(x) + " of cell " + std::to_string(c) + " may fire and is not in a pair unit";
                }
                if (seen_pair && !xp) order_ok = false;
                seen_pair = seen_pair || xp;
            }
            if ((t.lane_flags[s] & 1) && nx > 0) {
                if (!pair_u) return "cell " + std::to_string(c) + " may fire, has a neighbour that may, and sits in a single unit";
                if (!order_ok) return "chain of cell " + std::to_string(c) + ": a single unit's value behind a pair unit's";
            }
            const bool exit_want = pair_u && t.ds[c] >= 0 && slot_of[t.ds[c]] >= 0 && !(t.unit_p[slot_of[t.ds[c]] / LANES] & 16);
            if (((t.lane_flags[s] & 2) != 0) != exit_want) return "exit flag of cell " + std::to_string(c);
        }
        if (!t.fold_of_slot.empty() && t.fold_of_slot[s] >= 0) terms.push_back(t.fold_of_slot[s]);
        want.clear();
        for (int64_t j = indptr[c]; j < indptr[c + 1]; ++j) {
            if (indices[j] == c) {
                if (sign[j] >= 0) return "diagonal sign";
            } else {
                want.push_back(indices[j]);
            }
        }
        std::sort(terms.begin(), terms.end());
        std::sort(want.begin(), want.end());
        if (terms != want) return "inflow of cell " + std::to_string(c) + " does not expand to its upstream neighbours";
    }
    for (int c = 0; c < n; ++c) {
        if (!handled[c] || slot_of[c] < 0) continue;
        const int s = slot_of[c];
        const int want_readers = t.ds[c] >= 0 ? 1 : 0;
        const int have = readers_lane[s] + (t.export_edge[s] >= 0 ? 1 : 0);
        if (have != want_readers) return "cell " + std::to_string(c) + " has " + std::to_string(have) + " readers";
    }
    for (int ed = 0; ed < t.n_edges; ++ed)
        if (readers_ghost[ed] != 1) return "stream " + std::to_string(ed) + " has " + std::to_string(readers_ghost[ed]) + " readers";
    return "";
}
```

### xanthos_amd/csrc/xh_mrtm.hip

```cpp
#include <algorithm>
#include <chrono>
#include <climits>
#include <cmath>
#include <atomic>
#include <numeric>
#include <thread>

#include "xh_common.h"
#include <sys/stat.h>
#include <unistd.h>

#include "xh_mrtm_flow.h"
#include "xh_mrtm_plan.h"

namespace {

constexpr int W_MAX = 9;
constexpr int W_BASE = 3;
constexpr int UNIT_MAX_CELLS = 3072;
constexpr int BIN_CELLS = 256;
constexpr int N_CLASS = XH_ROUTE_N_CLASS;

struct UnitClass {
    int nt, kc;
// ... 698 lines not shown
    if (!plan || !n_words) return XH_ERR_ARG;
    std::vector<unsigned long long> st;
    const FlowPlan *rsum = last_reassoc(plan);
    int rc = flow_stats_fetch(plan->ctx, const_cast<FlowPlan *>(rsum ? rsum : plan->form[XH_FORM_EXACT].fp), st);
    if (rc) return rc;
    *n_words = (int64_t)st.size();
    if (h_words)
        for (int64_t i = 0; i < (int64_t)st.size() && i < max_words; ++i) h_words[i] = st[i];
    return XH_OK;
}

constexpr double CAPABLE_THRESHOLD = 1.0 - 1.0 / 1048576.0;

void xh_route_confirm(const xh_route_record &r) { r.plan->fault_streak = 0; }

extern "C" int xh_route_plan_prepare(xh_ctx *ctx, xh_route_plan *plan, const double *h_flow_dist, const double *h_velocity,
                                     double dt) {
    if (!ctx || !plan) return XH_ERR_ARG;
    XH_REQUIRE(ctx, plan->ctx == ctx, "xh_route_plan_prepare: plan belongs to another context");
    XH_REQUIRE(ctx, h_flow_dist && h_velocity && dt > 0.0, "xh_route_plan_prepare: bad argument");
    XH_HIP(ctx, hipSetDevice(ctx->device));
    if (reassoc_wanted(0)) {
        static const bool fold_on = xh_env_on("XH_FLOW_FOLD", true), single_on = xh_env_on("XH_RSUM_SINGLE", true);
        if ((!fold_on && !single_on) || !plan->form[XH_FORM_EXACT].fp || plan->h_indptr.empty()) return XH_OK;
        const size_t n = (size_t)plan->ncell;
        std::vector<unsigned char> foldable(n, 0), capable(n, 0);
        size_t nfold = 0;
        uint64_t key = XH_FNV_BASIS;
        for (size_t c = 0; c < n; ++c) {
            const double tauinv = h_velocity[c] / h_flow_dist[c];
            const bool leaf = plan->h_indptr[c + 1] - plan->h_indptr[c] == 1;
            capable[c] = (tauinv * dt <= CAPABLE_THRESHOLD) ? 0 : 1;
            foldable[c] = (leaf && tauinv >= 0.0 && tauinv * dt <= CAPABLE_THRESHOLD) ? 1 : 0;
            nfold += foldable[c];
            const unsigned char sets = (unsigned char)(capable[c] | (foldable[c] << 1));
            key = xh_fnv1a(key, &sets, 1);
        }
        key = xh_fnv1a(key, &dt, sizeof(dt));
        if (key == 0) key = 1;
        if (plan->fold_tried && key == plan->prep_key) return XH_OK;
        RouteForm &prepared = plan->form[XH_FORM_PREPARED];
        if (prepared.fp) {
            XH_HIP(ctx, hipStreamSynchronize(ctx->stream));
            if (plan->last.fp == prepared.fp) {
                plan->last.form = XH_FORM_EXACT;
                plan->last.fp = nullptr;
            }
            flow_plan_destroy(prepared.fp);
            prepared.fp = nullptr;
            prepared.first_checked = false;
        }
        plan->fold_tried = true;
        plan->prep_key = key;
        plan->fold_disabled = false;
        const bool fold = fold_on && nfold > 0;
        if (!fold && !single_on) return XH_OK;
        const int rcu = rsum_partition(ctx, plan, fold ? foldable.data() : nullptr, single_on ? capable.data() : nullptr,
                                       &prepared.fp);
        if (rcu || !prepared.fp) return rcu;
        prepared.suffix = prepared.fp->n_special >= 0 ? "_rs" : "_rf";
        plan->fold_dt = dt;
        return XH_OK;
    }
    return XH_OK;
}

void xh_route_backoff(xh_route_plan *plan) {
    plan->fault_streak = std::min(plan->fault_streak + 1, 6);
    plan->skip_calls = 4 << plan->fault_streak;
}

extern "C" int xh_route_plan_rsum_info(const xh_route_plan *plan, int64_t info[8]) {
    if (!plan || !info) return XH_ERR_ARG;
    const FlowPlan *fp = last_reassoc(plan), *prep = plan->form[XH_FORM_PREPARED].fp;
    info[0] = fp ? fp->n_units : 0;
    info[1] = fp ? fp->n_folded : 0;
    info[2] = plan->fold_disabled ? 1 : 0;
    info[3] = prep ? prep->n_folded : 0;
    info[4] = fp ? fp->n_special : -1;
    info[5] = prep ? prep->n_special : -1;
    info[6] = plan->guard_trips;
    info[7] = fp ? fp->n_pair_units : 0;
    return XH_OK;
}

RouteChoice route_choose(const xh_route_plan *plan, int flags, double dt, bool fed) {
    RouteChoice c;
    c.whole_graph = (flags & XH_ROUTE_FORCE_FALLBACK) != 0;
    c.atomic = (flags & XH_ROUTE_ATOMIC) != 0;
    c.dataflow = !c.whole_graph && plan->form[XH_FORM_EXACT].fp && (flags & XH_ROUTE_NO_DATAFLOW) == 0;
    c.skew = (flags & XH_ROUTE_NO_SKEW) == 0;
    c.checkable = c.dataflow && !c.atomic && (flags & XH_ROUTE_TEST_FAULT) == 0;
    if (c.dataflow && c.skew && !c.atomic && reassoc_wanted(flags) && !plan->rsum_failed) {
        c.form = XH_FORM_PAIRS;
        if (plan->form[XH_FORM_PREPARED].fp && !plan->fold_disabled && dt == plan->fold_dt && (flags & XH_ROUTE_NO_PLAIN) == 0)
            c.form = XH_FORM_PREPARED;
    }
    c.refuse_fed = fed && (!c.dataflow || !c.skew || c.atomic || plan->n_rest_units > 0 || plan->fb_rest.n > 0);
    return c;
}

int route_series_impl(xh_ctx *ctx, xh_route_plan *plan, int32_t nmonths, int32_t spinup_months,
                             const int32_t *h_ndays, double dt, const double *d_flow_dist, const double *d_velocity,
                             const double *d_area, const double *d_runoff, const double *d_S0, double *d_chstorage,
                             double *d_avgchflow, double *d_S_end, double *d_F_end, int32_t flags, xh_route_outcome *out,
                             const FlowFeed *feed) {
    if (!ctx || !plan) return XH_ERR_ARG;
    XH_REQUIRE(ctx, plan->ctx == ctx, "xh_route_series: plan belongs to another context");
    XH_REQUIRE(ctx, h_ndays && d_flow_dist && d_velocity && d_area && d_runoff, "xh_route_series: NULL argument");
    XH_REQUIRE(ctx, nmonths > 0 && spinup_months >= 0 && spinup_months <= nmonths,
               "xh_route_series: need 0 <= spinup_months (%d) <= nmonths (%d)", spinup_months, nmonths);
    XH_REQUIRE(ctx, dt > 0.0, "xh_route_series: dt must be positive");
    if (plan->ncell == 0) return XH_OK;

    const int nit = spinup_months + nmonths;
    std::vector<int> sm(nit), snt(nit);
    std::vector<double> ssecs(nit);
    std::vector<unsigned char> swr(nit);
    for (int it = 0; it < nit; ++it) {
        const int m = it < spinup_months ? it : it - spinup_months;
        XH_REQUIRE(ctx, h_ndays[m] > 0, "xh_route_series: ndays[%d] = %d", m, h_ndays[m]);
        sm[it] = m;
        ssecs[it] = (double)((int64_t)h_ndays[m] * 24 * 3600);
        snt[it] = (int)(ssecs[it] / dt);
        XH_REQUIRE(ctx, snt[it] >= 1, "xh_route_series: dt longer than a month");
        swr[it] = it >= spinup_months ? 1 : 0;
    }
    std::vector<int> sg(nit + 1, 0);
    for (int it = 0; it < nit; ++it) {
        XH_REQUIRE(ctx, (int64_t)sg[it] + snt[it] < (int64_t)1 << 30, "xh_route_series: more than 2^30 sub-steps");
        sg[it + 1] = sg[it] + snt[it];
    }
    const size_t sched_bytes = (size_t)nit * (3 * sizeof(int) + sizeof(double) + 1) + 64;
    void *sbuf = nullptr;
    int rc = xh_scratch(ctx, 2, sched_bytes, &sbuf);
    if (rc) return rc;
    double *d_secs = static_cast<double *>(sbuf);
    int *d_m = reinterpret_cast<int *>(d_secs + nit);
    int *d_nt = d_m + nit;
    int *d_g = d_nt + nit;
    unsigned char *d_wr = reinterpret_cast<unsigned char *>(d_g + nit + 1);
    bool sched_on_device = false;
    auto sched_upload = [&]() -> int {
        if (sched_on_device) return XH_OK;
        sched_on_device = true;
        XH_HIP(ctx, hipMemcpyAsync(d_secs, ssecs.data(), sizeof(double) * nit, hipMemcpyHostToDevice, ctx->stream));
        XH_HIP(ctx, hipMemcpyAsync(d_m, sm.data(), sizeof(int) * nit, hipMemcpyHostToDevice, ctx->stream));
        XH_HIP(ctx, hipMemcpyAsync(d_nt, snt.data(), sizeof(int) * nit, hipMemcpyHostToDevice, ctx->stream));
        XH_HIP(ctx, hipMemcpyAsync(d_g, sg.data(), sizeof(int) * (nit + 1), hipMemcpyHostToDevice, ctx->stream));
        XH_HIP(ctx, hipMemcpyAsync(d_wr, swr.data(), (size_t)nit, hipMemcpyHostToDevice, ctx->stream));
        return XH_OK;
    };
    *out = xh_route_outcome();
    RouteChoice c = route_choose(plan, flags, dt, feed != nullptr);
    if (c.form != XH_FORM_EXACT && !plan->form[XH_FORM_PAIRS].fp) {
        if ((rc = rsum_plan_build(ctx, plan)) != XH_OK) return rc;
        c = route_choose(plan, flags, dt, feed != nullptr);
    }
    if (c.refuse_fed) return XH_ERR_LIMIT;

    struct Span {
        xh_span s;
        bool open = true;
        ~Span() { if (open) xh_span_cancel(s); }
    } span{xh_span_begin(ctx, "mrtm_route")};
    if (!(c.dataflow && plan->n_rest_units == 0 && plan->fb_rest.n == 0) && (rc = sched_upload()) != XH_OK) return rc;
// ... 154 lines not shown
```

### xanthos_amd/csrc/xh_mrtm_check.hip

```cpp
#include <algorithm>
#include <cmath>

#include "xh_mrtm_plan.h"

__global__ void __launch_bounds__(256) k_count_diff(const unsigned long long *a, const unsigned long long *b, int64_t n,
                                                    unsigned long long *count) {
    unsigned long long local = 0;
    for (int64_t i = (int64_t)blockIdx.x * blockDim.x + threadIdx.x; i < n; i += (int64_t)gridDim.x * blockDim.x) {
        const double x = __longlong_as_double((long long)a[i]), y = __longlong_as_double((long long)b[i]);
        local += (x == y || (x != x && y != y)) ? 0ull : 1ull;
    }
    if (local) atomicAdd(count, local);
}

__global__ void __launch_bounds__(256) k_count_far(const double *a, const double *b, int64_t n, double rel, double tiny,
                                                   unsigned long long *count) {
    unsigned long long local = 0;
    for (int64_t i = (int64_t)blockIdx.x * blockDim.x + threadIdx.x; i < n; i += (int64_t)gridDim.x * blockDim.x) {
        const double x = a[i], y = b[i];
        const bool xn = x != x, yn = y != y;
        local += (xn || yn) ? (xn != yn ? 1ull : 0ull) : ((fabs(x - y) <= rel * fabs(y) + tiny) ? 0ull : 1ull);
    }
    if (local) atomicAdd(count, local);
}

static int route_validate(xh_ctx *ctx, xh_route_plan *plan, int32_t nmonths, int32_t spinup_months, const int32_t *h_ndays,
                          double dt, const double *d_flow_dist, const double *d_velocity, const double *d_area,
                          const double *d_runoff, const double *d_S0, const double *d_chs, const double *d_avg,
                          const double *d_S_end, const double *d_F_end, int32_t flags, bool by_rsum) {
    int rc = xh_settle(ctx);
    if (rc) return rc;
    const size_t nc = (size_t)plan->ncell, big = nc * (size_t)nmonths * sizeof(double);
    double *t_chs = nullptr, *t_avg = nullptr, *t_S = nullptr, *t_F = nullptr;
    unsigned long long *d_cnt = nullptr, h_cnt = 0;
    auto release = [&]() {
        for (void *p : {(void *)t_chs, (void *)t_avg, (void *)t_S, (void *)t_F, (void *)d_cnt})
            if (p) (void)hipFree(p);
    };
    hipError_t e = hipSuccess;
    if (d_chs) e = hipMalloc(reinterpret_cast<void **>(&t_chs), big);
    if (e == hipSuccess && d_avg) e = hipMalloc(reinterpret_cast<void **>(&t_avg), big);
    if (e == hipSuccess && d_S_end) e = hipMalloc(reinterpret_cast<void **>(&t_S), nc * sizeof(double));
    if (e == hipSuccess && d_F_end) e = hipMalloc(reinterpret_cast<void **>(&t_F), nc * sizeof(double));
    if (e == hipSuccess) e = hipMalloc(reinterpret_cast<void **>(&d_cnt), sizeof(unsigned long long));
    if (e != hipSuccess) {
        release();
        return xh_fail(ctx, XH_ERR_HIP, "XH_ROUTE_VALIDATE: no memory for the second set of outputs");
    }
    xh_route_outcome second;
    rc = route_series_impl(ctx, plan, nmonths, spinup_months, h_ndays, dt, d_flow_dist, d_velocity, d_area, d_runoff, d_S0,
                           t_chs, t_avg, t_S, t_F, (flags | XH_ROUTE_NO_DATAFLOW) & ~XH_ROUTE_TEST_FAULT, &second);
    if (!rc) {
        (void)hipMemsetAsync(d_cnt, 0, sizeof(unsigned long long), ctx->stream);
        auto cmp = [&](const double *a, const double *b, size_t n, double tiny) {
            if (!(a && b && n)) return;
            if (by_rsum)
                hipLaunchKernelGGL(k_count_far, dim3(1024), dim3(256), 0, ctx->stream, a, b, (int64_t)n, 1e-9, tiny, d_cnt);
            else
                hipLaunchKernelGGL(k_count_diff, dim3(1024), dim3(256), 0, ctx->stream,
                                   reinterpret_cast<const unsigned long long *>(a),
                                   reinterpret_cast<const unsigned long long *>(b), (int64_t)n, d_cnt);
        };
        cmp(d_chs, t_chs, nc * (size_t)nmonths, 1e-3);
        cmp(d_avg, t_avg, nc * (size_t)nmonths, 1e-9);
        cmp(d_S_end, t_S, nc, 1e-3);
        cmp(d_F_end, t_F, nc, 1e-9);
        if (hipMemcpyAsync(&h_cnt, d_cnt, sizeof(h_cnt), hipMemcpyDeviceToHost, ctx->stream) != hipSuccess ||
            hipStreamSynchronize(ctx->stream) != hipSuccess)
            rc = xh_fail(ctx, XH_ERR_HIP, "XH_ROUTE_VALIDATE: comparison failed to run");
    }
    release();
    if (rc) return rc;
    plan->validated += 1;
    if (h_cnt)
        return xh_fail(ctx, XH_ERR_DEVICE, "XH_ROUTE_VALIDATE: %llu output values of the dataflow routing kernel differ from "
                       "the workgroup-per-network kernel%s", h_cnt, by_rsum ? " by more than 1e-9 (reassociated form)" : "");
    return XH_OK;
}

static int route_series_call(xh_ctx *ctx, xh_route_plan *plan, int32_t nmonths, int32_t spinup_months,
                             const int32_t *h_ndays, double dt, const double *d_flow_dist,
                             const double *d_velocity, const double *d_area, const double *d_runoff,
                             const double *d_S0, double *d_chstorage, double *d_avgchflow, double *d_S_end,
                             double *d_F_end, int32_t flags, const FlowFeed *feed);

extern "C" int xh_route_series(xh_ctx *ctx, xh_route_plan *plan, int32_t nmonths, int32_t spinup_months,
                               const int32_t *h_ndays, double dt, const double *d_flow_dist,
                               const double *d_velocity, const double *d_area, const double *d_runoff,
                               const double *d_S0, double *d_chstorage, double *d_avgchflow, double *d_S_end,
                               double *d_F_end, int32_t flags) {
    return route_series_call(ctx, plan, nmonths, spinup_months, h_ndays, dt, d_flow_dist, d_velocity, d_area, d_runoff, d_S0,
                             d_chstorage, d_avgchflow, d_S_end, d_F_end, flags, nullptr);
}

int xh_route_series_fed(xh_ctx *ctx, xh_route_plan *plan, int32_t nmonths, int32_t spinup_months, const int32_t *h_ndays,
                        double dt, const double *d_flow_dist, const double *d_velocity, const double *d_area,
                        const double *d_runoff, const double *d_S0, double *d_chstorage, double *d_avgchflow,
                        int32_t flags, const FlowFeed *feed) {
    return route_series_call(ctx, plan, nmonths, spinup_months, h_ndays, dt, d_flow_dist, d_velocity, d_area, d_runoff, d_S0,
                             d_chstorage, d_avgchflow, nullptr, nullptr, flags, feed);
}

static std::string first_check_path(const xh_ctx *ctx, const xh_route_plan *plan, int form, bool for_write) {
    uint64_t h = xh_fnv1a(XH_FNV_BASIS, ctx->prop.name);
    h = xh_fnv1a(h, ctx->prop.gcnArchName);
    h = xh_fnv1a(h, __DATE__ " " __TIME__);
    {
        int rt = 0, drv = 0;
        (void)hipRuntimeGetVersion(&rt);
        (void)hipDriverGetVersion(&drv);
        char ver[96];
        const char *tag = getenv("XH_TEST_RUNTIME_TAG");
        snprintf(ver, sizeof(ver), "rt%d drv%d %s", rt, drv, tag ? tag : "");
        h = xh_fnv1a(h, ver);
    }
    char key[24] = "";
    if (form == XH_FORM_PREPARED) snprintf(key, sizeof(key), "_%016llx", (unsigned long long)plan->prep_key);
    char name[160];
    snprintf(name, sizeof(name), "route_ok_%016llx_%016llx_%lld_%lld%s%s", (unsigned long long)h, (unsigned long long)plan->topo_hash,
             (long long)plan->ncell, (long long)(plan->form[XH_FORM_EXACT].fp ? plan->form[XH_FORM_EXACT].fp->n_units : 0), key,
             plan->form[form].suffix);
    return xh_cache_path(name, for_write);
}

static bool first_check_needed(xh_ctx *ctx, xh_route_plan *plan, int form) {
    static const bool enabled = xh_env_on("XH_ROUTE_VALIDATE_FIRST", true);
    bool &checked = plan->form[form].first_checked;
    if (!enabled || checked || !plan->form[XH_FORM_EXACT].fp) return false;
    const std::string path = first_check_path(ctx, plan, form, false);
    if (!path.empty()) {
        if (FILE *f = fopen(path.c_str(), "r")) {
            fclose(f);
            checked = true;
            return false;
        }
    }
    return true;
}

static void first_check_passed(xh_ctx *ctx, xh_route_plan *plan, int form) {
    plan->form[form].first_checked = true;
    const std::string path = first_check_path(ctx, plan, form, true);
    if (path.empty()) return;
    if (FILE *f = fopen(path.c_str(), "w")) {
        fprintf(f, "dataflow routing equal to the workgroup-per-network kernel, %s, on %s\n", form ? "within 1e-9" : "bit for bit", ctx->prop.name);
        fclose(f);
    }
}

static int route_series_call(xh_ctx *ctx, xh_route_plan *plan, int32_t nmonths, int32_t spinup_months,
                             const int32_t *h_ndays, double dt, const double *d_flow_dist,
                             const double *d_velocity, const double *d_area, const double *d_runoff,
                             const double *d_S0, double *d_chstorage, double *d_avgchflow, double *d_S_end,
                             double *d_F_end, int32_t flags, const FlowFeed *feed) {
    if (!plan) return XH_ERR_ARG;
    if (plan->skip_calls > 0 && (flags & XH_ROUTE_TEST_FAULT) == 0) {
        if (!feed) plan->skip_calls -= 1;
        flags |= XH_ROUTE_NO_DATAFLOW;
    }
    static const bool validate_env = xh_env_on("XH_ROUTE_VALIDATE", false);
    bool validate = validate_env || (flags & XH_ROUTE_VALIDATE) != 0;
    flags &= ~XH_ROUTE_VALIDATE;
    const RouteChoice choice = route_choose(plan, flags, dt, feed != nullptr);
    bool first_check = feed && !validate && choice.checkable && first_check_needed(ctx, plan, choice.form);
    bool check_due = false;
    if (choice.checkable) {
        const char *ev = getenv("XH_ROUTE_VALIDATE_EVERY");
        const int64_t every = ev ? (int64_t)atoll(ev) : (int64_t)1000;
        if (plan->validate_due && !feed) {
            check_due = !validate;
            plan->validate_due = false;
        } else {
            plan->dataflow_calls += 1;
            if (!validate && !first_check && every > 0 && plan->dataflow_calls % every == 0) {
                check_due = true;
                plan->validate_due = feed != nullptr;
            }
        }
    }
    if (feed && (validate || first_check || check_due || choice.refuse_fed)) return XH_ERR_LIMIT;
    xh_route_outcome ran;
    int rc = route_series_impl(ctx, plan, nmonths, spinup_months, h_ndays, dt, d_flow_dist, d_velocity, d_area, d_runoff,
                               d_S0, d_chstorage, d_avgchflow, d_S_end, d_F_end, flags, &ran, feed);
    if (rc) return rc;
    plan->last = ran;
    if (!ran.kernel) return XH_OK;
    xh_route_record r;
    r.plan = plan;
    r.nmonths = nmonths;
// ... 52 lines not shown
```

### xanthos_amd/csrc/xh_mrtm_flow.h

```cpp
#pragma once
#include <functional>
#include <string>
#include <vector>

#include "xh_common.h"
#include "xh_flow_plan.h"

struct FlowBuf {
    void *p = nullptr;
};

struct FlowPlan {
    int n_units = 0, n_edges = 0, depth = 0, n_cells = 0, max_imports = 0, max_exports = 0;
    bool rsum = false;
    int max_cell = -1;
    FlowBuf d_cell_of_slot, d_ent, d_export_edge, d_ghost_edge, d_edge_cons_unit, d_unit_terms;
    bool skew_ok = false;
    int skew_lmax = 0;
    int skew_span = 1;
    FlowBuf d_lag, d_ghost_lag, d_ent2, d_eprev, d_unit_p, d_unit_lmax, d_unit_glmax, d_unit_order;
    void *d_x = nullptr;
    size_t x_bytes = 0;
    unsigned long long *d_stats = nullptr;
    void *d_skew_args = nullptr;
    std::vector<char> h_rec, h_fin;
    uint64_t rec_key = 0;
    FlowBuf d_fold_cell;
    int n_folded = 0;
    int n_special = -1;
    int n_pair_units = 0;
    FlowBuf d_lane_flags;
};

struct FlowSched {
    int nmonths, nit, ntmax, ntmin, total;
    const int *d_m, *d_nt;
    const int *d_g;
    const double *d_secs;
    const unsigned char *d_wr;
    double dt;
    bool test_fault;
    bool nt_even;
    const int *h_m, *h_nt, *h_g;
    const double *h_secs;
    const unsigned char *h_wr;
};

struct FlowFeed {
    const double *q_staged = nullptr;
    int64_t ncell = 0;
    const unsigned *months_ready = nullptr;
    unsigned ready_at_launch = 0;
    unsigned *place_epoch = nullptr;
    unsigned epoch = 0;
};

struct FlowIO {
    const double *flow_dist, *velocity, *area, *runoff, *S0;
    double *chs, *avg, *S_end, *F_end;
    const FlowFeed *feed = nullptr;
};

int flow_plan_build(xh_ctx *ctx, int n, const int64_t *indptr, const int32_t *indices, const int8_t *sign, uint64_t topo_hash,
                    const std::vector<int> &comp, int ncomp, std::vector<char> &handled, FlowPlan **out);
int flow_tables_cached(const char *name, int n, const int64_t *indptr, const int32_t *indices, const int8_t *sign, bool rsum,
                       bool folds, bool singles, FlowTables &t, std::vector<char> &handled,
                       const std::function<int(FlowTables &, std::vector<char> &)> &build);
FlowPlanOptions flow_plan_options(const xh_ctx *ctx);
int flow_tables_host(FlowPlanOptions opt, int n, const int64_t *indptr, const int32_t *indices, const int8_t *sign,
                     const std::vector<int> &comp, int ncomp, std::vector<char> &handled, FlowTables &t, std::string &err);
int flow_plan_upload(xh_ctx *ctx, const FlowTables &t, FlowPlan **out);
void flow_plan_destroy(FlowPlan *fp);
void flow_plan_info(const FlowPlan *fp, int64_t info[5]);
int flow_launch(xh_ctx *ctx, FlowPlan *fp, const FlowSched &s, const FlowIO &io, hipStream_t st);
int wave_launch(xh_ctx *ctx, FlowPlan *fp, const FlowSched &s, const FlowIO &io, hipStream_t st, unsigned **place);
const void *wave_rsum_kernel();
const void *wave_exact_kernel();
int flow_stats_fetch(xh_ctx *ctx, FlowPlan *fp, std::vector<unsigned long long> &out);
```

### xanthos_amd/csrc/xh_mrtm_flow.hip

```cpp

#include <algorithm>
#include <cmath>
#include <cstdlib>
#include <numeric>

#include "xh_flow_plan.h"
#include "xh_mrtm_flow.h"

namespace {

constexpr int W_MAX = 9;
constexpr int LANES = 64;
constexpr int NPAIR = 2 * LANES + 1;
constexpr int RING = 4;
constexpr int PF = 8;
constexpr unsigned FAULT_DATA_WAIT = 1, FAULT_RING_WAIT = 2;
constexpr unsigned FAULT_TEST = 99;
constexpr unsigned long long SPIN_LIMIT_TICKS = 500000000ull;

struct FlowArgs {
    const int *cell_of_slot;
    const unsigned *ent;
    const int *export_edge;
    const int *ghost_edge;
// ... 266 lines not shown
            err = "flow plan check: " + bad;
            return -1;
        }
    }
    return 0;
}

int flow_tables_cached(const char *name, int n, const int64_t *indptr, const int32_t *indices, const int8_t *sign, bool rsum,
                       bool folds, bool singles, FlowTables &t, std::vector<char> &handled,
                       const std::function<int(FlowTables &, std::vector<char> &)> &build) {
    const std::string path = name ? xh_cache_path(name, false) : std::string();
    if (!path.empty() && flow_tables_load(path.c_str(), t) && t.rsum == rsum && t.n_units > 0 &&
        (int64_t)t.cell_of_slot.size() == (int64_t)t.n_units * LANES && (folds || t.n_folded == 0) && (singles || t.n_special < 0)) {
        handled.assign((size_t)n, 0);
        bool ok = true;
        for (const std::vector<int> *cells : {&t.cell_of_slot, &t.fold_of_slot})
            for (int c : *cells) {
                if (c >= n) ok = false;
                else if (c >= 0) handled[c] = 1;
            }
        if (ok && (rsum ? flow_tables_check_rsum : flow_tables_check)(n, indptr, indices, sign, handled, t).empty()) return 0;
    }
    t = FlowTables();
    const int rc = build(t, handled);
    if (rc == 0 && t.n_units > 0 && !path.empty()) (void)flow_tables_save(t, xh_cache_path(name, true).c_str());
    return rc;
}

int flow_plan_build(xh_ctx *ctx, int n, const int64_t *indptr, const int32_t *indices, const int8_t *sign, uint64_t topo_hash,
                    const std::vector<int> &comp, int ncomp, std::vector<char> &handled, FlowPlan **out) {
    *out = nullptr;
    FlowTables t;
    std::string err;
    const FlowPlanOptions opt = flow_plan_options(ctx);
    char name[96] = "";
    if (xh_plan_cache_on() && n > 0 && !opt.debug) {
        const int knobs[5] = {opt.simds, opt.piece_cap, opt.chain, opt.cut_rule, opt.tlimit};
        const uint64_t h = xh_fnv1a(xh_fnv1a(topo_hash, knobs, sizeof(knobs)), __DATE__ " " __TIME__);
        snprintf(name, sizeof(name), "pairs_%016llx_%d.tables", (unsigned long long)h, n);
    }
    auto build = [&](FlowTables &bt, std::vector<char> &bh) {
        return flow_tables_host(opt, n, indptr, indices, sign, comp, ncomp, bh, bt, err);
    };
    if (flow_tables_cached(name[0] ? name : nullptr, n, indptr, indices, sign, false, false, false, t, handled, build) != 0)
        return xh_fail(ctx, XH_ERR_ARG, "%s", err.c_str());
    return flow_plan_upload(ctx, t, out);
}

int flow_plan_upload(xh_ctx *ctx, const FlowTables &t, FlowPlan **out) {
    *out = nullptr;
    if (t.n_units == 0) return XH_OK;
    FlowPlan *fp = new FlowPlan();
    fp->skew_ok = t.skew_ok;
    fp->skew_lmax = t.skew_lmax;
    fp->skew_span = t.skew_span;
    fp->n_units = t.n_units;
    fp->n_edges = t.n_edges;
    fp->depth = t.depth;
    fp->n_cells = t.n_cells;
    fp->max_imports = t.max_imports;
    fp->max_exports = t.max_exports;
    fp->rsum = t.rsum;
    for (int c : t.cell_of_slot) fp->max_cell = std::max(fp->max_cell, c);
    for (int c : t.fold_of_slot) fp->max_cell = std::max(fp->max_cell, c);
    int rc = put(ctx, fp->d_cell_of_slot, t.cell_of_slot);
    rc |= put(ctx, fp->d_ent, t.ent);
    rc |= put(ctx, fp->d_export_edge, t.export_edge);
    rc |= put(ctx, fp->d_ghost_edge, t.ghost_edge);
    rc |= put(ctx, fp->d_edge_cons_unit, t.edge_cons_unit);
    rc |= put(ctx, fp->d_unit_terms, t.unit_terms);
    rc |= put(ctx, fp->d_lag, t.lag);
    rc |= put(ctx, fp->d_ghost_lag, t.ghost_lag);
    rc |= put(ctx, fp->d_ent2, t.ent2);
    rc |= put(ctx, fp->d_eprev, t.eprev);
    rc |= put(ctx, fp->d_unit_p, t.unit_p);
    rc |= put(ctx, fp->d_unit_order, t.unit_order);
    rc |= put(ctx, fp->d_unit_lmax, t.unit_lmax);
    rc |= put(ctx, fp->d_unit_glmax, t.unit_glmax);
    rc |= put(ctx, fp->d_lane_flags, t.lane_flags);
    if (!t.fold_of_slot.empty()) rc |= put(ctx, fp->d_fold_cell, t.fold_of_slot);
    fp->n_folded = t.n_folded;
    fp->n_special = t.n_special;
    fp->n_pair_units = t.n_pair_units;
    if (rc) {
        flow_plan_destroy(fp);
        return XH_ERR_HIP;
    }
    *out = fp;
    return XH_OK;
}

int flow_stats_fetch(xh_ctx *ctx, FlowPlan *fp, std::vector<unsigned long long> &out) {
    out.clear();
    if (!fp || !fp->d_stats) return XH_OK;
    out.resize((size_t)fp->n_units * 6);
    XH_HIP(ctx, hipStreamSynchronize(ctx->stream));
    XH_HIP(ctx, hipMemcpy(out.data(), fp->d_stats, out.size() * 8, hipMemcpyDeviceToHost));
    return XH_OK;
}

int flow_launch(xh_ctx *ctx, FlowPlan *fp, const FlowSched &s, const FlowIO &io, hipStream_t st) {
    if (!fp || fp->n_units == 0) return XH_OK;
    const size_t x_streams = (size_t)std::max(fp->n_edges, 1) * RING * (size_t)s.ntmax * sizeof(double2);
    const size_t x_cnt = ((size_t)(fp->n_edges + fp->n_units) * sizeof(unsigned) + 255) & ~size_t(255);
    fp->rec_key = 0;
    if (x_streams + x_cnt > fp->x_bytes) {
        if (fp->d_x) {
            XH_HIP(ctx, hipStreamSynchronize(st));
            XH_HIP(ctx, hipFree(fp->d_x));
            fp->d_x = nullptr;
        }
        XH_HIP(ctx, hipMalloc(&fp->d_x, x_streams + x_cnt));
        fp->x_bytes = x_streams + x_cnt;
    }
    unsigned *cnt = reinterpret_cast<unsigned *>(static_cast<char *>(fp->d_x) + x_streams);
    XH_HIP(ctx, hipMemsetAsync(cnt, 0, x_cnt, st));

    const int cus = ctx->prop.multiProcessorCount > 0 ? ctx->prop.multiProcessorCount : 256;
    const int per_cu = (fp->n_units + cus - 1) / cus + 1;
    const size_t lds_static = 2 * (size_t)NPAIR * sizeof(double2);
    const size_t share = ((size_t)(160 * 1024) / (size_t)per_cu) & ~size_t(1023);
    size_t lds = share > lds_static + 1024 ? share - lds_static : 0;
    XH_HIP(ctx, hipFuncSetAttribute(reinterpret_cast<const void *>(&k_mrtm_flow), hipFuncAttributeMaxDynamicSharedMemorySize,
                                    (int)lds));
    int resident = 0;
    XH_HIP(ctx, hipOccupancyMaxActiveBlocksPerMultiprocessor(&resident, k_mrtm_flow, LANES, lds));
    if ((int64_t)(resident - 1) * cus < fp->n_units)
        return xh_fail(ctx, XH_ERR_LIMIT, "dataflow routing: %d units but only (%d - 1) x %d can be resident", fp->n_units,
                       resident, cus);

    FlowArgs a;
    a.cell_of_slot = static_cast<const int *>(fp->d_cell_of_slot.p);
    a.ent = static_cast<const unsigned *>(fp->d_ent.p);
    a.export_edge = static_cast<const int *>(fp->d_export_edge.p);
    a.ghost_edge = static_cast<const int *>(fp->d_ghost_edge.p);
    a.edge_cons_unit = static_cast<const int *>(fp->d_edge_cons_unit.p);
    a.unit_terms = static_cast<const int *>(fp->d_unit_terms.p);
    a.total_slots = (int64_t)fp->n_units * LANES;
    a.nmonths = s.nmonths;
    a.nit = s.nit;
    a.ntmax = s.ntmax;
    a.sched_m = s.d_m;
    a.sched_nt = s.d_nt;
    a.sched_secs = s.d_secs;
    a.sched_write = s.d_wr;
    a.dt = s.dt;
    a.dtinv = 1.0 / s.dt;
    a.flow_dist = io.flow_dist;
    a.velocity = io.velocity;
    a.area = io.area;
    a.runoff = io.runoff;
    a.S0 = io.S0;
    a.chs = io.chs;
    a.avg = io.avg;
    a.S_end = io.S_end;
    a.F_end = io.F_end;
    a.xbuf = static_cast<double2 *>(fp->d_x);
    a.ready = cnt;
    a.done = cnt + fp->n_edges;
    unsigned *fault = nullptr;
    int rc = xh_fault_word(ctx, &fault);
    if (rc) return rc;
    a.fault = fault;
    if (s.test_fault) XH_HIP(ctx, hipMemsetD32Async(reinterpret_cast<hipDeviceptr_t>(fault), (int)FAULT_TEST, 1, st));
    a.stats = nullptr;
    {
// ... 11 lines not shown
```

### xanthos_amd/csrc/xh_mrtm_rsum.hip

```cpp
#include <algorithm>
#include "xh_mrtm_wave_unit.h"

namespace {

__global__ void __launch_bounds__(LANES) __attribute__((amdgpu_waves_per_eu(2, 2))) k_mrtm_rsum(const WaveArgs *ap_) {
    WaveArgsK *ap = (WaveArgsK *)ap_;
    __shared__ __attribute__((aligned(16))) v2d lds[RING * NSLOT];
    __shared__ uint2 xtab[LANES];
    __shared__ unsigned qstage_sh[4 * LANES];
    __shared__ double fend_sh[2 * LANES];
    __shared__ int unit_sh, prio_sh;
    const int unit = wave_claim(ap, &unit_sh, &prio_sh);
    const int prio = prio_sh;
    if (unit < 0) return;
    if (A(months_ready)) {
        if (prio == 3) __builtin_amdgcn_s_setprio(3);
        else if (prio == 1) __builtin_amdgcn_s_setprio(1);
        else __builtin_amdgcn_s_setprio(2);
    } else if (prio == 3) {
        __builtin_amdgcn_s_setprio(3);
    }
    const int p = A(unit_p)[unit];
    const bool has_ghost = A(ghost_edge)[(int64_t)unit * LANES + threadIdx.x] >= 0;
    const bool g = __any(has_ghost), g2 = __any(has_ghost && threadIdx.x >= 8);
    const int nxo = __popcll(__ballot(A(export_edge)[(int64_t)unit * LANES + threadIdx.x] >= 0));
    const bool x = nxo > 0;
    char *l = reinterpret_cast<char *>(lds);
    __attribute__((address_space(3))) unsigned *qst = (__attribute__((address_space(3))) unsigned *)qstage_sh;
    __attribute__((address_space(3))) double *fnd = (__attribute__((address_space(3))) double *)fend_sh;
    fend_sh[threadIdx.x] = 0.0;
    fend_sh[LANES + threadIdx.x] = 0.0;
    if ((p & ~31) != 0x400) {
        if (threadIdx.x == 0) __hip_atomic_store(A(fault), FAULT_PLACE_WAIT, __ATOMIC_RELAXED, __HIP_MEMORY_SCOPE_AGENT);
        return;
    }
    bool bad = false;
#define XH_BY_OUTLETS(...)                                                                 \
    do {                                                                                   \
        if (nxo > 8) wave_unit<__VA_ARGS__, -1>(ap, l, xtab, qst, fnd, unit);              \
        else if (x) wave_unit<__VA_ARGS__, 1>(ap, l, xtab, qst, fnd, unit);                \
        else wave_unit<__VA_ARGS__, 0>(ap, l, xtab, qst, fnd, unit);                       \
    } while (0)
    if (p & 16) {
        if (!(p & 8) || (p & 4)) bad = true;
        else if (g2) XH_BY_OUTLETS(1, 0, 2, true, true, false, 2);
        else if (g) XH_BY_OUTLETS(1, 0, 1, true, true, false, 2);
        else XH_BY_OUTLETS(1, 0, 0, true, true, false, 2);
#undef XH_BY_OUTLETS
    } else if (p & 8) {
        if (p & 4) {
            if (g || !A(fold_cell)) bad = true;
            else wave_unit<1, 0, 0, true, true, true, 1>(ap, l, xtab, qst, fnd, unit);
        } else if (g2) wave_unit<1, 0, 2, true, true, false, 1>(ap, l, xtab, qst, fnd, unit);
        else if (g) wave_unit<1, 0, 1, true, true, false, 1>(ap, l, xtab, qst, fnd, unit);
        else if ((p & 2) || x) wave_unit<1, 0, 0, true, true, false, 1>(ap, l, xtab, qst, fnd, unit);
        else if (p & 1) wave_unit<1, 0, 0, false, true, false, 1>(ap, l, xtab, qst, fnd, unit);
        else wave_unit<0, 0, 0, false, true, false, 1>(ap, l, xtab, qst, fnd, unit);
    } else if (p & 4) {
        if (g || !A(fold_cell)) bad = true;
        else wave_unit<1, 0, 0, true, true, true>(ap, l, xtab, qst, fnd, unit);
    } else if (g2) wave_unit<1, 0, 2, true, true>(ap, l, xtab, qst, fnd, unit);
    else if (g) wave_unit<1, 0, 1, true, true>(ap, l, xtab, qst, fnd, unit);
    else if ((p & 2) || x) wave_unit<1, 0, 0, true, true>(ap, l, xtab, qst, fnd, unit);
    else if (p & 1) wave_unit<1, 0, 0, false, true>(ap, l, xtab, qst, fnd, unit);
    else wave_unit<0, 0, 0, false, true>(ap, l, xtab, qst, fnd, unit);
    if (bad && threadIdx.x == 0)
        __hip_atomic_store(A(fault), FAULT_PLACE_WAIT, __ATOMIC_RELAXED, __HIP_MEMORY_SCOPE_AGENT);
}
#undef A

}

const void *wave_rsum_kernel() { return reinterpret_cast<const void *>(&k_mrtm_rsum); }
```

### xanthos_amd/csrc/xh_mrtm_wave_launch.hip

```cpp
#include <algorithm>
#include "xh_mrtm_wave_unit.h"
#undef A

namespace {

__global__ void k_mrtm_wave_args(WaveArgs a, WaveArgs *dst, uint4 *cnt, unsigned cnt_vec) {
    if (threadIdx.x == 0) *dst = a;
    if (threadIdx.x == 0 && a.months_ready)
        __hip_atomic_store(const_cast<unsigned *>(a.months_ready), a.ready_at_launch, __ATOMIC_RELAXED, __HIP_MEMORY_SCOPE_AGENT);
    for (unsigned i = threadIdx.x; i < cnt_vec; i += blockDim.x) cnt[i] = make_uint4(0u, 0u, 0u, 0u);
}

}

int wave_launch(xh_ctx *ctx, FlowPlan *fp, const FlowSched &s, const FlowIO &io, hipStream_t st, unsigned **place) {
    if (!fp || fp->n_units == 0) return XH_OK;
    if (!fp->skew_ok || fp->max_imports > 8 * SK_R || fp->max_exports > 8 * SK_R || s.ntmin < fp->skew_lmax + 2 * GROUP) {
        if (xh_flow_debug())
            fprintf(stderr, "time-skewed kernel not used: skew_ok %d, imports %d, outlets %d, shortest month %d sub-steps, largest lag %d\n",
                    (int)fp->skew_ok, fp->max_imports, fp->max_exports, s.ntmin, fp->skew_lmax);
        return XH_ERR_LIMIT;
    }
    {
        uint64_t limit = (uint64_t)1 << 32;
// ... 66 lines not shown
                              (fp->rsum ? 2 * LANES * sizeof(unsigned) + LANES * sizeof(double) : 0);
    int n_excl = 0;
    if (fp->rsum && fp->n_special >= 0 && fp->n_pair_units > 0 && xh_env_on("XH_RSUM_EXCL", true))
        n_excl = std::min(fp->n_pair_units, 0xffff);
    int n_wg = 0, resident = 0;
    size_t lds = 0;
    {
        n_wg = fp->n_units + cus;
        if (n_wg > 8 * cus) n_wg = std::max(fp->n_units, 8 * cus);
        {
            const char *env = getenv("XH_FLOW_SPARE");
            if (env) n_wg = fp->n_units + std::max(atoi(env), 0);
        }
        const int per_cu = (n_wg + cus - 1) / cus + 3;
        const size_t share = ((size_t)(160 * 1024) / (size_t)per_cu) & ~size_t(1023);
        lds = share > lds_static + 1024 ? share - lds_static : 0;
        XH_HIP(ctx, hipFuncSetAttribute(kernel, hipFuncAttributeMaxDynamicSharedMemorySize, (int)lds));
        XH_HIP(ctx, hipOccupancyMaxActiveBlocksPerMultiprocessor(&resident, kernel, LANES, lds));
        if ((int64_t)(resident - 1) * cus < n_wg || n_wg > 8 * cus) return XH_ERR_LIMIT;
    }

    WaveArgs a;
    a.cell_of_slot = static_cast<const int *>(fp->d_cell_of_slot.p);
    a.lag = static_cast<const int *>(fp->d_lag.p);
    a.ghost_lag = static_cast<const int *>(fp->d_ghost_lag.p);
    a.export_edge = static_cast<const int *>(fp->d_export_edge.p);
    a.ghost_edge = static_cast<const int *>(fp->d_ghost_edge.p);
    a.edge_cons_unit = static_cast<const int *>(fp->d_edge_cons_unit.p);
    a.ent2 = static_cast<const unsigned *>(fp->d_ent2.p);
    a.eprev = static_cast<const unsigned *>(fp->d_eprev.p);
    a.unit_p = static_cast<const int *>(fp->d_unit_p.p);
    a.unit_order = static_cast<const int *>(fp->d_unit_order.p);
    a.n_units = fp->n_units;
    a.unit_lmax = static_cast<const int *>(fp->d_unit_lmax.p);
    a.unit_glmax = static_cast<const int *>(fp->d_unit_glmax.p);
    a.total_slots = (int64_t)fp->n_units * LANES;
    a.nmonths = s.nmonths;
    a.nit = s.nit;
    a.total = s.total;
    a.odd_ok = s.nt_even ? 0 : 1;
    a.rec = d_rec;
    a.fin = d_fin;
    a.lane_flags = static_cast<const unsigned char *>(fp->d_lane_flags.p);
    a.dt = s.dt;
    a.dtinv = 1.0 / s.dt;
    a.flow_dist = io.flow_dist;
    a.velocity = io.velocity;
    a.area = io.area;
    a.runoff = feed ? feed->q_staged : io.runoff;
    a.q_row_stride = feed ? 128u : (unsigned)s.nmonths * 8u;
    a.ready_at_launch = feed ? feed->ready_at_launch : UINT_MAX;
    a.months_ready = feed ? feed->months_ready : nullptr;
    a.place_epoch = feed ? feed->place_epoch : nullptr;
    a.epoch = feed ? feed->epoch : 0u;
    a.n_excl = n_excl;
    a.fenced = xh_env_on("XH_ROUTE_FENCED", false) ? 1 : 0;
    a.S0 = io.S0;
    a.chs = io.chs;
    a.avg = io.avg;
    a.S_end = io.S_end;
    a.F_end = io.F_end;
    a.xbuf = static_cast<char *>(fp->d_x);
    a.xbytes = (unsigned)x_streams;
    a.ring_mask_b = (unsigned)rs * 16u - 1u;
    a.rs = rs;
    a.ready = cnt;
    a.done = cnt + fp->n_edges;
    a.place = cnt + fp->n_edges + fp->n_units;
    *place = a.place;
    unsigned *fault = nullptr;
    int rc = xh_fault_word(ctx, &fault);
    if (rc) return rc;
    a.fault = fault;
    if (s.test_fault) XH_HIP(ctx, hipMemsetD32Async(reinterpret_cast<hipDeviceptr_t>(fault), (int)FAULT_TEST, 1, st));
    a.stats = nullptr;
    {
        const char *env = getenv("XH_FLOW_STATS");
        if (env && env[0] == '1') {
            if (!fp->d_stats) XH_HIP(ctx, hipMalloc(reinterpret_cast<void **>(&fp->d_stats), (size_t)fp->n_units * 48));
            a.stats = fp->d_stats;
        }
    }
    a.fold_cell = static_cast<const int *>(fp->d_fold_cell.p);
    if (!fp->d_skew_args) XH_HIP(ctx, hipMalloc(&fp->d_skew_args, sizeof(WaveArgs) + 256));
    hipLaunchKernelGGL(k_mrtm_wave_args, dim3(1), dim3(256), 0, st, a, static_cast<WaveArgs *>(fp->d_skew_args),
                       reinterpret_cast<uint4 *>(cnt), (unsigned)(x_cnt / sizeof(uint4)));
    {
        const WaveArgs *d_args = static_cast<const WaveArgs *>(fp->d_skew_args);
        void *kargs[] = {&d_args};
        XH_HIP(ctx, hipLaunchKernel(kernel, dim3((unsigned)n_wg), dim3(LANES), kargs, lds, st));
    }
    XH_HIP(ctx, hipGetLastError());
    return XH_OK;
}
```

### xanthos_amd/csrc/xh_mrtm_wave_unit.h

```cpp
#pragma once
#include <algorithm>
#include <climits>
#include <cstdlib>
#include <type_traits>

#include "xh_mrtm_flow.h"
#include "xh_mrtm_rec.h"

namespace {


constexpr int LANES = 64;
constexpr int SK_P = 4;
#ifndef XH_WAVE_MIDZONE
#define XH_WAVE_MIDZONE 1
#endif
#ifndef XH_WAVE_BMOV
#define XH_WAVE_BMOV 1
#endif
constexpr int NSLOT = 2 * LANES + 1;
constexpr int RING = 8;
constexpr int GROUP = 16;
constexpr int SK_R = 2;
#ifndef XH_WAVE_CH
#define XH_WAVE_CH 256
#endif
constexpr int CH = XH_WAVE_CH;
constexpr unsigned FAULT_DATA_WAIT = 1, FAULT_RING_WAIT = 2, FAULT_PLACE_WAIT = 3, FAULT_GUARD = XH_FAULT_GUARD;
constexpr unsigned FAULT_TEST = 99;
constexpr int PLACE_KEYS = 16 * 8 * 2 * 16 * 4;

constexpr int PLACE_WORDS = 16 + PLACE_KEYS + PLACE_KEYS / 4;

struct WaveArgs {
    const int *cell_of_slot, *lag, *ghost_lag, *export_edge, *ghost_edge, *edge_cons_unit;
    const unsigned *ent2;
    const unsigned *eprev;
    const int *unit_p, *unit_lmax, *unit_glmax;
    const unsigned char *lane_flags;
    int64_t total_slots;
    int nmonths, nit, total;
    const int *unit_order;
    unsigned *place;
    int n_units;
    int odd_ok;
    const MonthRec *rec;
    const FinRec *fin;
    double dt, dtinv;
    const double *flow_dist, *velocity, *area, *runoff, *S0;
    double *chs, *avg, *S_end, *F_end;
    unsigned q_row_stride;
    unsigned ready_at_launch;
    const unsigned *months_ready;
    unsigned *place_epoch;
    unsigned epoch;
    int n_excl;
    int fenced;
    char *xbuf;
    unsigned xbytes;
    unsigned ring_mask_b;
    int rs;
    unsigned *ready;
    unsigned *done;
    unsigned *fault;
    unsigned long long *stats;
    const int *fold_cell;
};

__device__ __forceinline__ unsigned ld_relaxed(const unsigned *p) {
    return __hip_atomic_load(p, __ATOMIC_RELAXED, __HIP_MEMORY_SCOPE_AGENT);
}

constexpr unsigned long long SPIN_LIMIT_TICKS = 500000000ull;

__device__ __forceinline__ bool wave_wait_ge(bool need, const unsigned *p, unsigned target, unsigned &seen,
                                             unsigned *fault, unsigned code) {
    bool ok = !need || seen >= target;
    if (__all(ok)) return true;
    const unsigned long long t0 = __builtin_amdgcn_s_memrealtime();
    for (;;) {
        if (!ok) {
            seen = ld_relaxed(p);
            ok = seen >= target;
        }
        if (__all(ok)) return true;
        if (ld_relaxed(fault) != 0) return false;
        if (__builtin_amdgcn_s_memrealtime() - t0 > SPIN_LIMIT_TICKS) {
            __hip_atomic_store(fault, code, __ATOMIC_RELAXED, __HIP_MEMORY_SCOPE_AGENT);
            return false;
        }
        __builtin_amdgcn_s_sleep(4);
    }
}

typedef double v2d __attribute__((ext_vector_type(2)));
typedef unsigned v4u __attribute__((ext_vector_type(4)));
constexpr int AUX_SC1 = 16;
typedef __attribute__((address_space(3))) const char lds_cchar;
typedef __attribute__((address_space(3))) char lds_char;

typedef __attribute__((address_space(4))) const WaveArgs WaveArgsK;
template <class T>
__device__ __forceinline__ T xh_ldarg(__attribute__((address_space(4))) const T *p) {
    asm volatile("" : "+s"(p));
    return *p;
}
#define A(f) xh_ldarg(&ap->f)

template <bool ONE> struct Val;
template <> struct Val<false> {
    typedef v2d T;
    typedef __attribute__((address_space(3))) const v2d lds_c;
    typedef __attribute__((address_space(3))) v2d lds_m;
    static constexpr unsigned B = 16;
    static __device__ __forceinline__ T zero() { return v2d{0.0, 0.0}; }
};
template <> struct Val<true> {
    typedef double T;
    typedef __attribute__((address_space(3))) const double lds_c;
    typedef __attribute__((address_space(3))) double lds_m;
    static constexpr unsigned B = 8;
    static __device__ __forceinline__ T zero() { return 0.0; }
};

template <int PRE, int POST, int NG, bool CHAIN, bool RSUM = false, bool FOLD = false, int SGL = 0, int NXR = -1>
__device__ __forceinline__ void wave_unit(WaveArgsK *ap, char *lds_generic, uint2 *xtab,
                                          __attribute__((address_space(3))) unsigned *qstage,
                                          __attribute__((address_space(3))) double *fend, const int unit) {
    constexpr bool HAS_G = NG > 0;
    constexpr bool V8 = SGL == 1;
    typedef Val<V8> V;
    typedef typename V::T val_t;
    typedef typename V::lds_c lds_cv;
    typedef typename V::lds_m lds_mv;
    constexpr unsigned VB = V::B;
    constexpr unsigned SLOTB = NSLOT * VB;
    lds_char *lds0 = (lds_char *)lds_generic;
    const int lane = threadIdx.x;
    const int64_t slot = (int64_t)unit * LANES + lane;

    const int gc = A(cell_of_slot)[slot];
    const bool valid = gc >= 0;
    const int gc_safe = valid ? gc : 0;
    const unsigned row_off = (unsigned)gc_safe * A(q_row_stride);
    const double tauinv = valid ? A(velocity)[gc] / A(flow_dist)[gc] : 0.0;
    const double acoef = 1.0 - tauinv * A(dt);
    const double area = valid ? A(area)[gc] : 0.0;
    const double S0v = (valid && A(S0)) ? A(S0)[gc] : 0.0;
    auto ent_off = [](unsigned o) { return V8 ? o >> 1 : o; };
    static_assert(!RSUM || (PRE <= 1 && POST == 0), "reassociated form: one inflow entry");
    static_assert(!FOLD || (RSUM && NG == 0), "folded leaves: reassociated form, units without imports");
    static_assert(SGL == 0 || RSUM, "single-sum plans: reassociated form");
    const int gcL = FOLD ? A(fold_cell)[slot] : -1;
    const bool validL = FOLD && valid && gcL >= 0;
    const unsigned row_offL = (unsigned)(validL ? gcL : 0) * A(q_row_stride);
    const double tauL = validL ? A(velocity)[gcL] / A(flow_dist)[gcL] : 0.0;
    const double acoefL = 1.0 - tauL * A(dt);
    const double areaL = validL ? A(area)[gcL] : 0.0;
    const double S0L = (validL && A(S0)) ? A(S0)[gcL] : 0.0;
    double SL = 0.0, favgL = 0.0, erlL = 0.0, erlL_n = 0.0, snapSL = 0.0, snapAL = 0.0, FL = 0.0;
    constexpr double FOLD_EPS = 1e-6;
    unsigned gfold = (validL && !(tauL * A(dt) <= 1.0 - 1.0 / 1048576.0 && tauL >= 0.0 && S0L >= 0.0)) ? 1u : 0u;
    constexpr double SGL_EPS = 1e-6;
    constexpr double SGL_XEPS = 1e-10;
    unsigned gsgl = 0;
    bool xlane = false;
    double fmin_seen = 0.0;
    if (SGL != 0) {
        const unsigned lf = A(lane_flags)[slot];
        xlane = valid && (lf & 2u) != 0;
        gsgl = (valid && (!(tauinv >= 0.0) || (!(tauinv * A(dt) <= 1.0 - 1.0 / 1048576.0) && !(lf & 1u)) || S0v < 0.0)) ? 1u : 0u;
    }
    constexpr int PRE_N = PRE > 0 ? PRE : 1, POST_N = POST > 0 ? POST : 1;
    lds_cchar *epre[PRE_N], *epost[POST_N];
#pragma unroll
    for (int w = 0; w < PRE; ++w) epre[w] = lds0 + ent_off(A(ent2)[(int64_t)w * A(total_slots) + slot]);
#pragma unroll
    for (int w = 0; w < POST; ++w) epost[w] = lds0 + ent_off(A(ent2)[(int64_t)(SK_P + w) * A(total_slots) + slot]);
    lds_cchar *eprv = lds0 + (CHAIN ? ent_off(A(eprev)[slot]) : 0u);
    lds_mv *own = (lds_mv *)lds0 + lane;
    const int xedge = A(export_edge)[slot];
    const int gedge = A(ghost_edge)[slot];
    const bool has_x = xedge >= 0, has_g = gedge >= 0;
    const unsigned long long xmask = __ballot(has_x), gmask = __ballot(has_g);
    const int nx_out = __popcll(xmask), ng = __popcll(gmask);
    static_assert(NXR >= -1 && NXR <= 1, "outlet rounds known at compile time: none or one");
    const bool any_x = NXR < 0 ? xmask != 0 : NXR > 0, any_g = HAS_G;
    const int lmax = A(unit_lmax)[unit], glmax = A(unit_glmax)[unit];
    const int lag_g = has_g ? A(ghost_lag)[slot] : 0;
    const unsigned *ready_p = A(ready) + (has_g ? gedge : 0);
    const unsigned *done_p = A(done) + (has_x ? A(edge_cons_unit)[xedge] : 0);
    const unsigned maskb = A(ring_mask_b);
    const unsigned oob = ~maskb;
    const __amdgpu_buffer_rsrc_t xr = __builtin_amdgcn_make_buffer_rsrc(A(xbuf), 0, (int)A(xbytes), 0x00020000);
    const int total = A(total), nit = A(nit);
    const bool odd_ok = A(odd_ok) != 0;

    if (has_x) xtab[__popcll(xmask & ((1ull << lane) - 1ull))] = make_uint2((unsigned)lane, (unsigned)xedge);
    const int sub = lane & 7, grp = lane >> 3;
    const bool x2 = NXR < 0 && nx_out > 8;
    unsigned gfull[SK_R], xbyte[SK_R];
    lds_mv *gdst[SK_R];
    lds_cv *xsrc[SK_R];
#pragma unroll
    for (int r = 0; r < SK_R; ++r) {
        const int k = r * 8 + grp;
        const bool gon = k < ng, xon = k < nx_out;
        const int ge = gon ? A(ghost_edge)[(int64_t)unit * LANES + k] : 0;
        const int gl = gon ? A(ghost_lag)[(int64_t)unit * LANES + k] : 0;
        gfull[r] = gon ? ((unsigned)ge * (maskb + 1u)) | (((unsigned)(sub - gl) * 16u) & maskb) : oob;
        gdst[r] = (lds_mv *)(lds0 + sub * SLOTB) + LANES + (k & 63);
        const uint2 t = xon ? xtab[k] : make_uint2((unsigned)lane, 0u);
        xbyte[r] = xon ? t.y * (maskb + 1u) + (unsigned)sub * 16u : oob;
        xsrc[r] = (lds_cv *)(lds0 + sub * SLOTB) + t.x;
    }
#pragma unroll
    for (int k = 0; k < RING; ++k) {
        own[k * NSLOT] = V::zero();
        own[k * NSLOT + LANES] = V::zero();
        if (lane == 0) own[k * NSLOT + 2 * LANES] = V::zero();
    }

    const double dt = A(dt), dtinv = A(dtinv);
    double S = 0.0, F = 0.0, favg = 0.0, erl = 0.0;
    double snapS = 0.0, snapA = 0.0;
    int nx = A(lag)[slot];
    const double *p_runoff = A(runoff);
    double *p_chs = A(chs), *p_avg = A(avg);
    typedef __attribute__((address_space(4))) const MonthRec MonthRecK;
    MonthRecK *p_rec = (MonthRecK *)A(rec);
    typedef __attribute__((address_space(4))) const FinRec FinRecK;
    FinRecK *p_fin = (FinRecK *)A(fin);
    auto ld_fin = [&](int i) {
        FinRec r = {};
        r.m_prev_w = p_fin[i].m_prev_w;
        r.m_next2 = p_fin[i].m_next2;
        r.g_next1 = p_fin[i].g_next1;
        r.q_off_next2 = p_fin[i].q_off_next2;
        r.nt_cur = p_fin[i].nt_cur;
        if constexpr (RSUM) {
            r.erl_scale_next1 = p_fin[i].erl_scale_next1;
            r.inv_nt_prev = p_fin[i].inv_nt_prev;
        } else {
            r.nt_prev = p_fin[i].nt_prev;
            r.secs_next1 = p_fin[i].secs_next1;
        }
        return r;
    };
    FinRec fc = ld_fin(0);
    auto ld_rec = [&](int i) {
// ... 4 lines not shown
        r.write = p_rec[i].write;
        r.secs = p_rec[i].secs;
        r.q_off = p_rec[i].q_off;
        return r;
    };
    const int nmo = A(nmonths);
    const unsigned q_lds = (unsigned)(size_t)qstage;
    auto runoff_fetch = [&](long long q_off) {
        const char *src = reinterpret_cast<const char *>(p_runoff) + q_off + (size_t)row_off;
        unsigned keep;
        asm volatile("s_mov_b32 %0, m0\n\ts_mov_b32 m0, %2\n\tglobal_load_lds_dword %1, off\n\ts_add_u32 m0, m0, 252\n\t"
                     "global_load_lds_dword %1, off offset:4\n\ts_mov_b32 m0, %0"
                     : "=&s"(keep)
                     : "v"(src), "s"(q_lds)
                     : "memory");
        if (FOLD) {
            const char *srcL = reinterpret_cast<const char *>(p_runoff) + q_off + (size_t)row_offL;
            asm volatile("s_mov_b32 %0, m0\n\ts_mov_b32 m0, %2\n\tglobal_load_lds_dword %1, off\n\ts_add_u32 m0, m0, 252\n\t"
                         "global_load_lds_dword %1, off offset:4\n\ts_mov_b32 m0, %0"
                         : "=&s"(keep)
                         : "v"(srcL), "s"(q_lds + 2u * LANES * 4u)
                         : "memory");
        }
    };
    auto runoff_take = [&]() {
        if (any_x || any_g) asm volatile("s_waitcnt vmcnt(4)" ::: "memory");
        else asm volatile("s_waitcnt vmcnt(0)" ::: "memory");
        const unsigned lo = qstage[lane], hi = qstage[LANES + lane];
        return __hiloint2double((int)hi, (int)lo);
    };
    double erl_n = 0.0;
    {
        const MonthRec r0 = ld_rec(0), r1 = ld_rec(1);
        auto ld_q = [&](long long q_off) {
            return *reinterpret_cast<const double *>(reinterpret_cast<const char *>(p_runoff) + q_off + (size_t)row_off);
        };
        const double q0 = ld_q(r0.q_off);
        if constexpr (RSUM) {
            const double scale0 = 1000.0 * A(dt) / r0.secs;
            erl_n = ((valid ? q0 : 0.0) * area) * scale0;
            if (FOLD) {
                const double q0L = *reinterpret_cast<const double *>(reinterpret_cast<const char *>(p_runoff) + r0.q_off + (size_t)row_offL);
                erlL_n = ((validL ? q0L : 0.0) * areaL) * scale0;
            }
        } else {
            erl_n = ((valid ? q0 : 0.0) * area) * 1000.0 / r0.secs;
        }
        if (SGL != 0) gsgl |= (erl_n < -SGL_EPS) ? 2u : 0u;
        if (nit > 1) runoff_fetch(r1.q_off);
    }
    constexpr int OB = 4;
    double ob_s[OB], ob_a[OB];
    double ob_sL[FOLD ? OB : 1], ob_aL[FOLD ? OB : 1];
#pragma unroll
    for (int j = 0; j < OB; ++j) ob_s[j] = ob_a[j] = 0.0;
#pragma unroll
    for (int j = 0; j < (FOLD ? OB : 1); ++j) ob_sL[j] = ob_aL[j] = 0.0;
    bool alive = true;
    unsigned mready = A(ready_at_launch);
    auto wait_months = [&](unsigned need) {
        const unsigned *p = A(months_ready);
        if (!p) return true;
        const unsigned long long t0 = __builtin_amdgcn_s_memrealtime();
        for (;;) {
            unsigned v = 0;
            if (lane == 0) v = __hip_atomic_fetch_add(const_cast<unsigned *>(p), 0u, __ATOMIC_RELAXED, __HIP_MEMORY_SCOPE_AGENT);
            v = (unsigned)__builtin_amdgcn_readfirstlane((int)v);
            if (v >= need) {
                mready = v;
                return true;
            }
            if (ld_relaxed(A(fault)) != 0) return false;
            if (__builtin_amdgcn_s_memrealtime() - t0 > SPIN_LIMIT_TICKS) {
                __hip_atomic_store(A(fault), FAULT_DATA_WAIT, __ATOMIC_RELAXED, __HIP_MEMORY_SCOPE_AGENT);
                return false;
            }
            __builtin_amdgcn_s_sleep(16);
        }
    };
    unsigned long long cyc_wait_data = 0, cyc_wait_ring = 0, zone_groups = 0;
    const unsigned long long cyc_begin = __builtin_amdgcn_s_memtime();
    const unsigned long long rt_begin = __builtin_amdgcn_s_memrealtime();

    unsigned seen_ready = 0, seen_done = 0, pend_ready = 0, pend_done = 0;
    auto load_async = [&](const unsigned *q) {
        unsigned v;
        asm volatile("global_load_dword %0, %1, off sc1" : "=v"(v) : "v"(q) : "memory");
        return v;
    };
    auto check = [&](int n) {
        const unsigned long long w0 = __builtin_amdgcn_s_memtime();
        asm volatile("s_waitcnt vmcnt(8)" : "+v"(pend_ready), "+v"(pend_done) : : "memory");
        asm volatile("s_waitcnt vmcnt(0)" ::: "memory");
        if (SGL == 2) gsgl |= (xlane && fmin_seen < -SGL_XEPS) ? 4u : 0u;
        if ((FOLD && __any(gfold != 0)) || (SGL != 0 && __any(gsgl != 0))) {
            __hip_atomic_store(A(fault), FAULT_GUARD, __ATOMIC_RELAXED, __HIP_MEMORY_SCOPE_AGENT);
            alive = false;
        }
        const bool fenced = A(fenced) == 1;
        if (any_x) {
            const int pub = min(max(n - RING - lmax, 0), total);
            if (fenced) __builtin_amdgcn_fence(__ATOMIC_RELEASE, "agent");
            if (has_x) __hip_atomic_store(A(ready) + xedge, (unsigned)pub, __ATOMIC_RELAXED, __HIP_MEMORY_SCOPE_AGENT);
            const int need = n + CH - lmax - A(rs);
            seen_done = max(seen_done, pend_done);
            if (need > 0 && alive)
                alive = wave_wait_ge(has_x, done_p, (unsigned)min(need, total), seen_done, A(fault), FAULT_RING_WAIT);
        }
        const unsigned long long w1 = __builtin_amdgcn_s_memtime();
        if (any_g && alive) {
            if (lane == 0)
                __hip_atomic_store(A(done) + unit, (unsigned)min(max(n - glmax, 0), total), __ATOMIC_RELAXED,
                                   __HIP_MEMORY_SCOPE_AGENT);
            const int need = min(total, n + CH + GROUP - lag_g);
            seen_ready = max(seen_ready, pend_ready);
            alive = wave_wait_ge(has_g && need > 0, ready_p, (unsigned)max(need, 0), seen_ready, A(fault), FAULT_DATA_WAIT);
            if (fenced) __builtin_amdgcn_fence(__ATOMIC_ACQUIRE, "agent");
            asm volatile("" ::: "memory");
        }
        if (any_x) pend_done = load_async(done_p);
        if (any_g) pend_ready = load_async(ready_p);
        cyc_wait_ring += w1 - w0;
        cyc_wait_data += __builtin_amdgcn_s_memtime() - w1;
    };

    auto finalize = [&](int it) {
        const FinRec f = fc;
        fc = ld_fin(it + 1 <= nit ? it + 1 : nit + 1);
        if (it + 1 < nit) {
            const double qn = runoff_take();
            if constexpr (RSUM) erl_n = ((valid ? qn : 0.0) * area) * f.erl_scale_next1;
            else erl_n = ((valid ? qn : 0.0) * area) * 1000.0 / f.secs_next1;
            if (SGL != 0) gsgl |= (erl_n < -SGL_EPS) ? 2u : 0u;
            if (FOLD) {
                const unsigned lo = qstage[2 * LANES + lane], hi = qstage[3 * LANES + lane];
                const double qnL = __hiloint2double((int)hi, (int)lo);
                erlL_n = ((validL ? qnL : 0.0) * areaL) * f.erl_scale_next1;
            }
        }
        if (it >= 1) {
            const int m = f.m_prev_w & (FIN_WRITE - 1);
            const bool write_prev = (f.m_prev_w & FIN_WRITE) != 0;
#pragma unroll
            for (int j = 0; j < OB - 1; ++j) {
                ob_s[j] = ob_s[j + 1];
                ob_a[j] = ob_a[j + 1];
            }
            ob_s[OB - 1] = snapS;
            if constexpr (RSUM) ob_a[OB - 1] = snapA * f.inv_nt_prev;
            else ob_a[OB - 1] = snapA / (double)f.nt_prev;
            if (FOLD) {
#pragma unroll
                for (int j = 0; j < OB - 1; ++j) {
                    ob_sL[j] = ob_sL[j + 1];
                    ob_aL[j] = ob_aL[j + 1];
                }
                ob_sL[OB - 1] = snapSL;
                ob_aL[OB - 1] = snapAL * f.inv_nt_prev;
                gfold |= (snapSL < -FOLD_EPS) ? 2u : 0u;
                if (write_prev && validL) {
                    if ((m & (OB - 1)) == OB - 1) {
                        const int64_t o = (int64_t)gcL * nmo + (m - (OB - 1));
#pragma unroll
                        for (int j = 0; j < OB; j += 2) {
                            if (p_chs) *reinterpret_cast<v2d *>(p_chs + o + j) = v2d{ob_sL[j], ob_sL[j + 1]};
                            if (p_avg) *reinterpret_cast<v2d *>(p_avg + o + j) = v2d{ob_aL[j], ob_aL[j + 1]};
                        }
                    } else if (m == nmo - 1) {
                        const int r = (m & (OB - 1)) + 1;
                        const int64_t o = (int64_t)gcL * nmo + (m + 1 - r);
#pragma unroll
                        for (int j = 0; j < OB; ++j)
                            if (j >= OB - r) {
                                if (p_chs) p_chs[o + j - (OB - r)] = ob_sL[j];
                                if (p_avg) p_avg[o + j - (OB - r)] = ob_aL[j];
                            }
                    }
                }
            }
            if (write_prev && valid) {
                if ((m & (OB - 1)) == OB - 1) {
                    const int64_t o = (int64_t)gc * nmo + (m - (OB - 1));
#pragma unroll
                    for (int j = 0; j < OB; j += 2) {
                        if (p_chs) *reinterpret_cast<v2d *>(p_chs + o + j) = v2d{ob_s[j], ob_s[j + 1]};
                        if (p_avg) *reinterpret_cast<v2d *>(p_avg + o + j) = v2d{ob_a[j], ob_a[j + 1]};
                    }
                } else if (m == nmo - 1) {
                    const int r = (m & (OB - 1)) + 1;
                    const int64_t o = (int64_t)gc * nmo + (m + 1 - r);
#pragma unroll
                    for (int j = 0; j < OB; ++j)
                        if (j >= OB - r) {
                            if (p_chs) p_chs[o + j - (OB - r)] = ob_s[j];
                            if (p_avg) p_avg[o + j - (OB - r)] = ob_a[j];
                        }
                }
            }
        }
        if (it + 2 < nit) {
            if ((unsigned)f.m_next2 >= mready) alive = wait_months((unsigned)f.m_next2 + 1u);
            if (alive) runoff_fetch(f.q_off_next2);
        }
    };

    val_t va[2][PRE_N], vb[2][POST_N], vr[2];
    v4u gbuf[2][SK_R];
#pragma unroll
    for (int q = 0; q < 2; ++q) {
#pragma unroll
        for (int w = 0; w < PRE; ++w) va[q][w] = V::zero();
#pragma unroll
        for (int w = 0; w < POST; ++w) vb[q][w] = V::zero();
        vr[q] = V::zero();
    }
    auto import_load = [&](int r) {
        const v4u v = __builtin_amdgcn_raw_buffer_load_b128(xr, gfull[r], 0, AUX_SC1);
        gfull[r] = (gfull[r] & ~maskb) | ((gfull[r] + RING * 16u) & maskb);
        return v;
    };
    auto import_drop = [&](int r, const v4u u) {
        if (SGL == 1) {
            typedef unsigned v2u __attribute__((ext_vector_type(2)));
            *reinterpret_cast<__attribute__((address_space(3))) v2u *>(gdst[r]) = v2u{u.z, u.w};
        } else {
            *reinterpret_cast<__attribute__((address_space(3))) v4u *>(gdst[r]) = u;
        }
    };
    val_t xb[SK_R];
#pragma unroll
    for (int r = 0; r < SK_R; ++r) {
        xb[r] = V::zero();
    }
    auto block_io = [&](const int b) {
        if (HAS_G) {
#pragma unroll
            for (int r = 0; r < NG; ++r) {
                import_drop(r, gbuf[b][r]);
                gbuf[b][r] = import_load(r);
            }
        }
        if (any_x) {
            xb[0] = *xsrc[0];
            if (x2) xb[1] = *xsrc[1];
        }
    };
    auto store_pair = [&](const val_t v, unsigned voff, unsigned soff) {
        v2d p;
        if constexpr (SGL == 1) p = v2d{v, v};
        else p = v;
        __builtin_amdgcn_raw_buffer_store_b128(__builtin_bit_cast(v4u, p), xr, voff, soff, AUX_SC1);
    };
    auto block_store = [&](int m0) {
        if (any_x) {
            const unsigned xpos = ((unsigned)(m0 - RING - lmax) * 16u) & maskb;
            store_pair(xb[0], xbyte[0], xpos);
            if (x2) store_pair(xb[1], xbyte[1], xpos);
        }
    };

    check(0);
#pragma unroll
    for (int r = 0; r < SK_R; ++r) gbuf[0][r] = r < NG ? import_load(r) : v4u{0u, 0u, 0u, 0u};
#pragma unroll
    for (int r = 0; r < SK_R; ++r) gbuf[1][r] = r < NG ? import_load(r) : v4u{0u, 0u, 0u, 0u};

    const int N = (total + lmax + 1 + GROUP - 1) & ~(GROUP - 1);
    int itz = 0, gz = 0;
    int nf = (lmax + 1 + GROUP - 1) & ~(GROUP - 1);

    auto substep = [&](auto zone_c, auto mid_c, const int n, const int j, const int edge, const int rel) {
        constexpr bool MID = decltype(mid_c)::value;
        if (decltype(zone_c)::value && ((j & 1) == 0 || (!MID && odd_ok))) {
            const bool c = rel == j;
#if XH_WAVE_BMOV
            {
                const unsigned long long cm = __ballot(c);
                unsigned long long sv;
                asm volatile("s_and_saveexec_b64 %[sv], %[cm]\n\tv_mov_b64 %[ss], %[s]\n\tv_mov_b64 %[sa], %[fa]\n\t"
                             "v_mov_b64 %[fa], 0\n\tv_mov_b64 %[e], %[en]\n\ts_mov_b64 exec, %[sv]"
                             : [ss] "+v"(snapS), [sa] "+v"(snapA), [fa] "+v"(favg), [e] "+v"(erl), [sv] "=&s"(sv)
                             : [s] "v"(S), [en] "v"(erl_n), [cm] "s"(cm)
                             : "scc");
            }
#else
            snapS = c ? S : snapS;
            snapA = c ? favg : snapA;

            favg = c ? 0.0 : favg;
            erl = c ? erl_n : erl;
#endif
            if (FOLD) {
                snapSL = c ? SL : snapSL;
                snapAL = c ? favgL : snapAL;
                favgL = c ? 0.0 : favgL;
                erlL = c ? erlL_n : erlL;
            }
            if (!MID) {
                if (edge == 1) S = c ? S0v : S;
                if (FOLD && edge == 1) SL = c ? S0L : SL;
                if (edge == 2) {
                    if (c) fend[lane] = F;
                    if (FOLD && c) fend[LANES + lane] = FL;
                }
            }
        }
        __builtin_amdgcn_sched_barrier(0);
        val_t(&ac)[PRE_N] = va[j & 1], (&bc)[POST_N] = vb[j & 1], (&an)[PRE_N] = va[(j & 1) ^ 1], (&bn)[POST_N] = vb[(j & 1) ^ 1];
        const val_t rc = vr[j & 1];
        const unsigned so = (unsigned)((j + RING - 1) & (RING - 1)) * SLOTB;
        if (CHAIN) vr[(j & 1) ^ 1] = *(lds_cv *)(eprv + so);
#pragma unroll
        for (int w = 0; w < PRE; ++w) an[w] = *(lds_cv *)(epre[w] + so);
#pragma unroll
        for (int w = 0; w < POST; ++w) bn[w] = *(lds_cv *)(epost[w] + so);
        __builtin_amdgcn_sched_barrier(0);
        __builtin_amdgcn_s_waitcnt(0xC07F | ((PRE + POST + (CHAIN ? 1 : 0) + 1) << 8));
        __builtin_amdgcn_sched_barrier(0);
        if ((j & (RING - 1)) == 0) block_io(j / RING);
        if ((j & (RING - 1)) == 1) block_store(n + j - 1);
        const double F0 = S * tauinv;
        if constexpr (RSUM) {
            double base = __builtin_fma(S, acoef, erl);
            if (FOLD) {
                FL = SL * tauL;
                SL = __builtin_fma(SL, acoefL, erlL);
                favgL += FL;
                base = __builtin_fma(FL, dt, base);
            }
            if constexpr (SGL == 1) {
                const double S1 = PRE ? __builtin_fma(ac[0], dt, base) : base;
                const double m = __builtin_fmin(S1, 0.0);
                const double f2 = __builtin_fma(m, dtinv, F0);
                own[(j & (RING - 1)) * NSLOT] = CHAIN ? rc + f2 : f2;
                S = S1 - m;
                F = f2;
                favg += f2;
            } else {
            const double S1 = PRE ? __builtin_fma(ac[0].x, dt, base) : base;
            const double S2 = PRE ? __builtin_fma(ac[0].y, dt, base) : base;
            const bool sx = S1 < 0.0;
            const double f2 = __builtin_fma(__builtin_fmin(S1, 0.0), dtinv, F0);
            own[(j & (RING - 1)) * NSLOT] = CHAIN ? v2d{rc.x + F0, rc.y + f2} : v2d{F0, f2};
            double Sn = S2;
            asm volatile("" : "+v"(Sn));
            S = sx ? 0.0 : Sn;
            F = f2;
            favg += f2;
            if (SGL == 2) fmin_seen = __builtin_fmin(fmin_seen, f2);
            }
        } else {
            double s1 = 0.0, s2 = 0.0;
#pragma unroll
            for (int w = 0; w < PRE; ++w) {
                s1 += ac[w].x;
                s2 += ac[w].y;
            }
            s1 -= F0;
#pragma unroll
            for (int w = 0; w < POST; ++w) s1 += bc[w].x;
            const double dsdt = s1 + erl;
            const bool sx = (dsdt * dt) < (-S);
            const double f2 = sx ? (dsdt + F0) + S * dtinv : F0;
            own[(j & (RING - 1)) * NSLOT] = CHAIN ? v2d{rc.x + F0, rc.y + f2} : v2d{F0, f2};
            s2 -= f2;
#pragma unroll
            for (int w = 0; w < POST; ++w) s2 += bc[w].y;
            const double dsdt2 = s2 + erl;
            double Sn = S + dsdt2 * dt;
            asm volatile("" : "+v"(Sn));
            S = sx ? 0.0 : Sn;
            F = f2;
            favg += f2;
        }
    };

#ifdef XH_WAVE_PROFILE
    unsigned long long prof_zone = 0, prof_fin = 0, prof_check = 0, prof_zx = 0, prof_hk = 0, prof_t = __builtin_amdgcn_s_memtime();
#define PROF_MARK(acc)                                                  \
    {                                                                   \
        const unsigned long long now_ = __builtin_amdgcn_s_memtime();   \
        acc += now_ - prof_t;                                           \
        prof_t = now_;                                                  \
    }
    unsigned long long prof_plain = 0;
#else
#define PROF_MARK(acc)
#endif
    int n = 0;
    for (;;) {
        PROF_MARK(prof_hk)
        if (n > 0 && n < N && (n & (CH - 1)) == 0) {
            check(n);
            PROF_MARK(prof_check)
        }
        if (alive && n == nf) {
            nx = itz < nit ? nx + fc.nt_cur : INT_MAX;
            gz = itz < nit ? fc.g_next1 : INT_MAX;
            PROF_MARK(prof_zx)
            finalize(itz);
            ++itz;
            nf = itz <= nit ? ((gz + lmax + 1 + GROUP - 1) & ~(GROUP - 1)) : INT_MAX;
            PROF_MARK(prof_fin)
        }
        if (n >= N || !alive) break;
        const int stop = min(N, (n | (CH - 1)) + 1);
        PROF_MARK(prof_hk)
        if (n + GROUP > gz) {
            const int edge = itz == 0 ? 1 : (itz == nit ? 2 : 0);
            const int n_end = min(nf, stop);
            auto zone_run = [&](auto mid_c) {
                do {
                    ++zone_groups;
                    const int rel = nx - n;
#pragma unroll
                    for (int j = 0; j < GROUP; ++j) substep(std::true_type(), mid_c, n, j, edge, rel);
                    n += GROUP;
                    PROF_MARK(prof_zone)
                } while (n < n_end);
            };
#if XH_WAVE_MIDZONE
            if (edge == 0 && !odd_ok) zone_run(std::true_type());
            else zone_run(std::false_type());
#else
            zone_run(std::false_type());
#endif
        } else {
            const int n_end = min(stop, gz & ~(GROUP - 1));
            do {
#pragma unroll
                for (int j = 0; j < GROUP; ++j) substep(std::false_type(), std::false_type(), n, j, 0, 0);
                n += GROUP;
                PROF_MARK(prof_plain)
            } while (n < n_end);
        }
    }
    if (alive) {
        if (SGL == 2) gsgl |= (xlane && fmin_seen < -SGL_XEPS) ? 4u : 0u;
        if ((FOLD && __any(gfold != 0)) || (SGL != 0 && __any(gsgl != 0))) {
            __hip_atomic_store(A(fault), FAULT_GUARD, __ATOMIC_RELAXED, __HIP_MEMORY_SCOPE_AGENT);
            alive = false;
        }
    }
    if (alive) {
        if (any_x) {
            const unsigned xpos = ((unsigned)(N - RING - lmax) * 16u) & maskb;
            store_pair(*xsrc[0], xbyte[0], xpos);
            if (x2) store_pair(*xsrc[1], xbyte[1], xpos);
            asm volatile("s_waitcnt vmcnt(0)" ::: "memory");
            if (A(fenced) == 1) __builtin_amdgcn_fence(__ATOMIC_RELEASE, "agent");
            if (has_x) __hip_atomic_store(A(ready) + xedge, (unsigned)total, __ATOMIC_RELAXED, __HIP_MEMORY_SCOPE_AGENT);
        }
        if (any_g && lane == 0)
            __hip_atomic_store(A(done) + unit, (unsigned)total, __ATOMIC_RELAXED, __HIP_MEMORY_SCOPE_AGENT);
        if (valid) {
            if (A(S_end)) A(S_end)[gc] = snapS;
            if (A(F_end)) A(F_end)[gc] = fend[lane];
        }
        if (validL) {
            if (A(S_end)) A(S_end)[gcL] = snapSL;
            if (A(F_end)) A(F_end)[gcL] = fend[LANES + lane];
        }
    }
    const bool guard_set = __any((gfold | gsgl) != 0);
    if (A(stats) && lane == 0) {
        unsigned long long *st = A(stats) + (int64_t)unit * 6;
        const unsigned long long cyc = __builtin_amdgcn_s_memtime() - cyc_begin;
        st[0] = cyc - cyc_wait_data - cyc_wait_ring;
        st[1] = cyc;
        st[2] = __builtin_amdgcn_s_memrealtime() - rt_begin;
        const unsigned hw = __builtin_amdgcn_s_getreg((4) | (0 << 6) | (31 << 11));
        const unsigned xcc = __builtin_amdgcn_s_getreg((20) | (0 << 6) | (3 << 11));
        st[3] = (unsigned long long)((PRE + POST + (CHAIN ? 1 : 0) + 1) & 15) | (any_g ? 16u : 0u) | (any_x ? 32u : 0u) |
                (V8 ? 64u : 0u) | (guard_set ? 128u : 0u) | ((unsigned long long)hw << 8) | ((unsigned long long)(xcc & 15u) << 40) |
                (zone_groups << 44);
        st[4] = cyc_wait_data;
        st[5] = cyc_wait_ring;
#ifdef XH_WAVE_PROFILE
        st[0] = prof_plain;
        st[4] = prof_zone;
        st[1] = (cyc & 0xffffffffull) | ((cyc_wait_data + cyc_wait_ring) << 32);
        st[2] = (prof_check << 32) | (prof_hk & 0xffffffffull);
        st[5] = (prof_fin << 32) | (prof_zx & 0xffffffffull);
        if (FOLD) st[3] |= 1ull << 63;
#endif
    }
}


__device__ __forceinline__ int wave_claim(WaveArgsK *ap, int *unit_sh_p, int *prio_sh_p) {
    int &unit_sh = *unit_sh_p, &prio_sh = *prio_sh_p;
    if (threadIdx.x == 0) {
        prio_sh = 0;
        unsigned *pl = A(place);
        const unsigned hw = __builtin_amdgcn_s_getreg((4) | (0 << 6) | (31 << 11));
        const unsigned xcc = __builtin_amdgcn_s_getreg((20) | (0 << 6) | (3 << 11)) & 15u;
        const unsigned key = ((((xcc * 8u + ((hw >> 13) & 7u)) * 2u + ((hw >> 12) & 1u)) * 16u + ((hw >> 8) & 15u)) * 4u) +
                             ((hw >> 4) & 3u);
        unsigned *pl_cu = pl + 16 + PLACE_KEYS + (key >> 2);
        const int n_units = A(n_units);
        const unsigned n_wg = gridDim.x;
        unsigned *fault = A(fault);
        auto wait_for = [&](unsigned *word, unsigned target) {
            const unsigned long long t0 = __builtin_amdgcn_s_memrealtime();
            while (__hip_atomic_load(word, __ATOMIC_ACQUIRE, __HIP_MEMORY_SCOPE_AGENT) < target) {
                if (ld_relaxed(fault) != 0 || __builtin_amdgcn_s_memrealtime() - t0 > SPIN_LIMIT_TICKS) {
                    __hip_atomic_store(fault, FAULT_PLACE_WAIT, __ATOMIC_RELAXED, __HIP_MEMORY_SCOPE_AGENT);
                    return false;
                }
                __builtin_amdgcn_s_sleep(8);
            }
            return true;
        };
        auto add = [&](int word) { return __hip_atomic_fetch_add(pl + word, 1u, __ATOMIC_RELAXED, __HIP_MEMORY_SCOPE_AGENT); };
        const unsigned rank = __hip_atomic_fetch_add(pl + 16 + key, 1u, __ATOMIC_RELAXED, __HIP_MEMORY_SCOPE_AGENT) & 0xffffu;
        bool leader = false;
        unsigned cu_rank = 0;
        if (rank == 0) {
            add(2);
            cu_rank = __hip_atomic_fetch_add(pl_cu, 1u, __ATOMIC_RELAXED, __HIP_MEMORY_SCOPE_AGENT) & 0xffffu;
            leader = cu_rank == 0u;
            if (leader) add(9);
        } else if (rank == 1) {
            add(1);
        }
        const unsigned registered = __hip_atomic_fetch_add(pl + 0, 1u, __ATOMIC_RELEASE, __HIP_MEMORY_SCOPE_AGENT);
        if (registered + 1u == n_wg && A(place_epoch))
            __hip_atomic_store(A(place_epoch), A(epoch), __ATOMIC_RELAXED, __HIP_MEMORY_SCOPE_AGENT);
        int idx = -1;
        if (wait_for(pl + 0, n_wg)) {
            const int firsts = (int)ld_relaxed(pl + 2), seconds = (int)ld_relaxed(pl + 1), leaders = (int)ld_relaxed(pl + 9);
            const int n_excl = A(n_excl);
            int ncu = min(n_excl, leaders);
            ncu = max(min(ncu, (seconds - max(n_units - firsts, 0)) / 7), 0);
            bool excl_cu = false;
            int displaced = 0, claimed = 0;
            bool ok = true;
            if (ncu > 0) {
                if (leader) {
                    if ((int)add(10) < ncu) {
                        const int cnt = (int)(ld_relaxed(pl_cu) & 0xffffu);
                        const int base = (int)add(13);
                        if (base < n_excl) {
                            __hip_atomic_fetch_or(pl_cu, 0x10000u, __ATOMIC_RELAXED, __HIP_MEMORY_SCOPE_AGENT);
                            __hip_atomic_fetch_add(pl + 11, (unsigned)(cnt - 1), __ATOMIC_RELAXED, __HIP_MEMORY_SCOPE_AGENT);
                            idx = n_units - 1 - base;
                        }
                    }
                    __hip_atomic_fetch_add(pl + 12, 1u, __ATOMIC_RELEASE, __HIP_MEMORY_SCOPE_AGENT);
                }
                ok = wait_for(pl + 12, (unsigned)leaders);
                excl_cu = (ld_relaxed(pl_cu) & 0x10000u) != 0;
                displaced = (int)ld_relaxed(pl + 11);
                claimed = min((int)ld_relaxed(pl + 13), n_excl);
            }
            const int nx = claimed;
            const int firsts_eff = firsts - displaced;
            const int need2 = max(n_units - firsts_eff, 0);
// ... 34 lines not shown
```

Before: 3.252 billion.

## Add linear-unit fast path for single-sum routing units that cannot fire

The planner marks single-sum units whose cells can never fire as linear and sets a shape bit. A new LIN template specialization of wave_unit runs a simpler recurrence for them: it tracks storage only, derives flow as S*tauinv, and guards against negative storage instead of doing the per-step clamp. Single units are also specialised by outlet count, and the asynchronous readiness-counter loads are replaced with synchronous loads inside check. The intent is fewer operations in the serial per-month chain, at the cost of more kernel variants and a small change in rounding.

```diff
diff --git a/include/xanthos_hip.h b/include/xanthos_hip.h
--- a/include/xanthos_hip.h
+++ b/include/xanthos_hip.h
@@ -145,6 +145,7 @@
 #define XH_ROUTE_REASSOC 128
 #define XH_ROUTE_EXACT 256
 int xh_route_plan_rsum_info(const xh_route_plan *plan, int64_t info[8]);
+int64_t xh_route_plan_linear_units(const xh_route_plan *plan);
 int xh_route_series(xh_ctx *ctx, xh_route_plan *plan, int32_t nmonths, int32_t spinup_months,
                     const int32_t *h_ndays, double dt,
                     const double *d_flow_dist, const double *d_velocity, const double *d_area,
diff --git a/xanthos_amd/_hip.py b/xanthos_amd/_hip.py
--- a/xanthos_amd/_hip.py
+++ b/xanthos_amd/_hip.py
@@ -133,6 +133,7 @@
     'xh_route_plan_info': (c_int, [_P, POINTER(c_int64)]),
     'xh_route_plan_stats': (c_int, [_P, c_int64, _P, POINTER(c_int64)]),
     'xh_route_plan_rsum_info': (c_int, [_P, POINTER(c_int64)]),
+    'xh_route_plan_linear_units': (c_int64, [_P]),
     'xh_route_plan_prepare': (c_int, [_P, _P, _P, _P, c_double]),
     'xh_mrtm_downstream': (c_int, [c_int64, c_int32, c_int32, _P, _P, _P, _P, _P]),
     'xh_mrtm_upstream': (c_int, [c_int64, c_int32, c_int32, _P, _P, _P, _P, _P]),
@@ -202,6 +203,7 @@
 _lib = None
 
 
+OPTIONAL_SYMBOLS = frozenset(['xh_route_plan_linear_units'])
 ABI_VERSION = 7
 
 
@@ -220,6 +222,8 @@
             try:
                 fn = getattr(handle, name)
             except AttributeError:
+                if name in OPTIONAL_SYMBOLS:
+                    continue
                 raise HipUnavailable('{} lacks {}: it was built from older sources; rebuild it (make -C xanthos_amd/csrc)'
                                      .format(LIB_PATH, name))
             fn.restype = res
@@ -827,8 +831,11 @@
     def rsum_info(self):
         arr = (c_int64 * 8)()
         self.ctx._check(lib().xh_route_plan_rsum_info(self.handle, arr))
-        return dict(zip(('units', 'folded', 'fold_disabled', 'prepared_folded', 'pair_cells', 'prepared_pair_cells', 'guard_trips',
-                         'pair_units'), list(arr)))
+        out = dict(zip(('units', 'folded', 'fold_disabled', 'prepared_folded', 'pair_cells', 'prepared_pair_cells', 'guard_trips',
+                        'pair_units'), list(arr)))
+        fn = getattr(lib(), 'xh_route_plan_linear_units', None)
+        out['linear_units'] = int(fn(self.handle)) if fn is not None else 0
+        return out
 
     def stats(self):
         n = c_int64(0)
diff --git a/xanthos_amd/csrc/xh_flow_plan.cpp b/xanthos_amd/csrc/xh_flow_plan.cpp
--- a/xanthos_amd/csrc/xh_flow_plan.cpp
+++ b/xanthos_amd/csrc/xh_flow_plan.cpp
@@ -921,7 +921,7 @@
 }
 
 namespace {
-constexpr unsigned long long TABLES_MAGIC = 0x3472546c66485806ull;
+constexpr unsigned long long TABLES_MAGIC = 0x3472546c66485807ull;
 
 template <class T>
 bool put_vec(FILE *f, const std::vector<T> &v) {
@@ -943,13 +943,14 @@
 }
 template <class F>
 bool tables_io(FILE *f, FlowTables &t, bool write, F &&vec) {
-    int head[13] = {t.n_units, t.n_edges, t.depth, t.n_cells, t.max_imports, t.max_exports, t.skew_ok ? 1 : 0,
-                    t.skew_lmax, t.skew_span, t.rsum ? 1 : 0, t.n_folded, t.n_special, t.n_pair_units};
+    int head[14] = {t.n_units, t.n_edges, t.depth, t.n_cells, t.max_imports, t.max_exports, t.skew_ok ? 1 : 0,
+                    t.skew_lmax, t.skew_span, t.rsum ? 1 : 0, t.n_folded, t.n_special, t.n_pair_units, t.n_linear_units};
     if (write ? fwrite(head, sizeof(head), 1, f) != 1 : fread(head, sizeof(head), 1, f) != 1) return false;
     if (!write) {
         t.n_units = head[0], t.n_edges = head[1], t.depth = head[2], t.n_cells = head[3], t.max_imports = head[4];
         t.max_exports = head[5], t.skew_ok = head[6] != 0, t.skew_lmax = head[7];
         t.skew_span = head[8], t.rsum = head[9] != 0, t.n_folded = head[10], t.n_special = head[11], t.n_pair_units = head[12];
+        t.n_linear_units = head[13];
     }
     return vec(t.cell_of_slot) && vec(t.export_edge) && vec(t.ghost_edge) && vec(t.edge_cons_unit) && vec(t.unit_terms) &&
            vec(t.ent) && vec(t.lag) && vec(t.ghost_lag) && vec(t.unit_p) && vec(t.unit_lmax) && vec(t.unit_glmax) &&
diff --git a/xanthos_amd/csrc/xh_flow_plan.h b/xanthos_amd/csrc/xh_flow_plan.h
--- a/xanthos_amd/csrc/xh_flow_plan.h
+++ b/xanthos_amd/csrc/xh_flow_plan.h
@@ -34,6 +34,7 @@
     std::vector<int> fold_of_slot;
     int n_folded = 0;
     int n_special = -1;
+    int n_linear_units = 0;
     int n_pair_units = 0;
 };
 
diff --git a/xanthos_amd/csrc/xh_flow_rsum.cpp b/xanthos_amd/csrc/xh_flow_rsum.cpp
--- a/xanthos_amd/csrc/xh_flow_rsum.cpp
+++ b/xanthos_amd/csrc/xh_flow_rsum.cpp
@@ -345,7 +345,7 @@
 
 }
 
-int flow_rsum_planner_version() { return 8; }
+int flow_rsum_planner_version() { return 9; }
 
 int flow_tables_build_rsum(int n, const int64_t *indptr, const int32_t *indices, const int8_t *sign, const int *comp,
                            int ncomp, const FlowPlanOptions &opt, std::vector<char> &handled, FlowTables &out,
@@ -538,6 +538,18 @@
             out.lane_flags[sl] = (unsigned char)((P.mayfire[c] ? 1 : 0) | ((P.special[c] && ds[c] >= 0 && !P.special[ds[c]]) ? 2 : 0));
         }
 
+    out.n_linear_units = 0;
+    if (P.n_special >= 0)
+        for (int u = 0; u < nunit; ++u) {
+            if (out.unit_p[u] & 16) continue;
+            bool any = false;
+            for (int k = 0; k < LANES && !any; ++k) any = (out.lane_flags[(int64_t)u * LANES + k] & 1) != 0;
+            if (!any) {
+                out.unit_p[u] |= 32;
+                out.n_linear_units++;
+            }
+        }
+
     std::vector<int> unit_exp(nunit, 0);
     for (int ed = 0; ed < nedge; ++ed) unit_exp[unit_of_piece[piece[P.e_prod[ed]]]]++;
     {
@@ -613,8 +625,8 @@
                 if (out.unit_p[u] & 16)
                     fprintf(stderr, "  pair unit %d: %d cells, %d imports, %d outlets, depth %d, lmax %d\n", u, P.unit_cells[u], P.unit_imp[u], unit_exp[u],
                             P.unit_depth[u], out.unit_lmax[u]);
-            fprintf(stderr, "  single-sum plan: %s, %d cells may fire, %d of them in pair form in %d units; %d single units hold no cell that may fire\n",
-                    P.n_special >= 0 ? "yes" : "no", nx, std::max(P.n_special, 0), nsu, quiet);
+            fprintf(stderr, "  single-sum plan: %s, %d cells may fire, %d of them in pair form in %d units; %d single units hold no cell that may fire (%d marked linear)\n",
+                    P.n_special >= 0 ? "yes" : "no", nx, std::max(P.n_special, 0), nsu, quiet, out.n_linear_units);
         }
         fprintf(stderr, "  units by reads (none, A, R, A+R): %d %d %d %d\n  units by lmax/16 (0..13+):", hs[0], hs[1], hs[2], hs[3]);
         for (int k = 0; k < 14; ++k) fprintf(stderr, " %d", hl[k]);
@@ -696,7 +708,8 @@
             }
         if (g != imp[u]) return "ghost count";
         if (t.unit_lmax[u] & 15) return "unit lag not a multiple of 16";
-        if ((t.unit_p[u] & ~31) != 0x400) return "shape word of unit " + std::to_string(u);
+        if ((t.unit_p[u] & ~63) != 0x400) return "shape word of unit " + std::to_string(u);
+        if ((t.unit_p[u] & 32) && (t.unit_p[u] & 24) != 8) return "linear flag of unit " + std::to_string(u) + " that is not a single unit";
         if (t.n_special >= 0 ? !(t.unit_p[u] & 8) : (t.unit_p[u] & 24) != 0) return "single-sum flags of unit " + std::to_string(u);
     }
     std::vector<int> readers_lane(ts, 0), readers_ghost(t.n_edges, 0);
@@ -752,6 +765,7 @@
         if (t.n_special >= 0) {
             if ((int64_t)t.lane_flags.size() != ts) return "lane flags";
             const bool pair_u = (t.unit_p[u] & 16) != 0;
+            if ((t.unit_p[u] & 32) && (t.lane_flags[s] & 1)) return "cell " + std::to_string(c) + " of a linear unit may fire";
             if (pair_u && !(t.lane_flags[s] & 1)) return "cell " + std::to_string(c) + " of a pair unit is not one that may fire";
             if (pair_u && !t.fold_of_slot.empty() && t.fold_of_slot[s] >= 0) return "folded leaf in a pair unit";
             int nx = 0;
diff --git a/xanthos_amd/csrc/xh_mrtm.hip b/xanthos_amd/csrc/xh_mrtm.hip
--- a/xanthos_amd/csrc/xh_mrtm.hip
+++ b/xanthos_amd/csrc/xh_mrtm.hip
@@ -804,6 +804,11 @@
     info[6] = plan->guard_trips;
     info[7] = fp ? fp->n_pair_units : 0;
     return XH_OK;
+}
+
+extern "C" int64_t xh_route_plan_linear_units(const xh_route_plan *plan) {
+    const FlowPlan *fp = plan ? last_reassoc(plan) : nullptr;
+    return fp && xh_env_on("XH_RSUM_LINEAR", true) ? fp->n_linear_units : 0;
 }
 
 RouteChoice route_choose(const xh_route_plan *plan, int flags, double dt, bool fed) {
diff --git a/xanthos_amd/csrc/xh_mrtm_check.hip b/xanthos_amd/csrc/xh_mrtm_check.hip
--- a/xanthos_amd/csrc/xh_mrtm_check.hip
+++ b/xanthos_amd/csrc/xh_mrtm_check.hip
@@ -105,6 +105,10 @@
     uint64_t h = xh_fnv1a(XH_FNV_BASIS, ctx->prop.name);
     h = xh_fnv1a(h, ctx->prop.gcnArchName);
     h = xh_fnv1a(h, __DATE__ " " __TIME__);
+    {
+        const int pv = flow_rsum_planner_version();
+        h = xh_fnv1a(h, &pv, sizeof(pv));
+    }
     {
         int rt = 0, drv = 0;
         (void)hipRuntimeGetVersion(&rt);
diff --git a/xanthos_amd/csrc/xh_mrtm_flow.h b/xanthos_amd/csrc/xh_mrtm_flow.h
--- a/xanthos_amd/csrc/xh_mrtm_flow.h
+++ b/xanthos_amd/csrc/xh_mrtm_flow.h
@@ -28,6 +28,7 @@
     FlowBuf d_fold_cell;
     int n_folded = 0;
     int n_special = -1;
+    int n_linear_units = 0;
     int n_pair_units = 0;
     FlowBuf d_lane_flags;
 };
diff --git a/xanthos_amd/csrc/xh_mrtm_flow.hip b/xanthos_amd/csrc/xh_mrtm_flow.hip
--- a/xanthos_amd/csrc/xh_mrtm_flow.hip
+++ b/xanthos_amd/csrc/xh_mrtm_flow.hip
@@ -372,6 +372,7 @@
     fp->n_folded = t.n_folded;
     fp->n_special = t.n_special;
     fp->n_pair_units = t.n_pair_units;
+    fp->n_linear_units = t.n_linear_units;
     if (rc) {
         flow_plan_destroy(fp);
         return XH_ERR_HIP;
diff --git a/xanthos_amd/csrc/xh_mrtm_rsum.hip b/xanthos_amd/csrc/xh_mrtm_rsum.hip
--- a/xanthos_amd/csrc/xh_mrtm_rsum.hip
+++ b/xanthos_amd/csrc/xh_mrtm_rsum.hip
@@ -2,6 +2,10 @@
 #include "xh_mrtm_wave_unit.h"
 
 namespace {
+
+#ifndef XH_RSUM_SINGLE_NXR
+#define XH_RSUM_SINGLE_NXR 1
+#endif
 
 __global__ void __launch_bounds__(LANES) __attribute__((amdgpu_waves_per_eu(2, 2))) k_mrtm_rsum(const WaveArgs *ap_) {
     WaveArgsK *ap = (WaveArgsK *)ap_;
@@ -30,32 +34,55 @@
     __attribute__((address_space(3))) double *fnd = (__attribute__((address_space(3))) double *)fend_sh;
     fend_sh[threadIdx.x] = 0.0;
     fend_sh[LANES + threadIdx.x] = 0.0;
-    if ((p & ~31) != 0x400) {
+    if ((p & ~63) != 0x400) {
         if (threadIdx.x == 0) __hip_atomic_store(A(fault), FAULT_PLACE_WAIT, __ATOMIC_RELAXED, __HIP_MEMORY_SCOPE_AGENT);
         return;
     }
     bool bad = false;
-#define XH_BY_OUTLETS(...)                                                                 \
+#define XH_BY_OUTLETS(LIN_, ...)                                                           \
     do {                                                                                   \
-        if (nxo > 8) wave_unit<__VA_ARGS__, -1>(ap, l, xtab, qst, fnd, unit);              \
-        else if (x) wave_unit<__VA_ARGS__, 1>(ap, l, xtab, qst, fnd, unit);                \
-        else wave_unit<__VA_ARGS__, 0>(ap, l, xtab, qst, fnd, unit);                       \
+        if (nxo > 8) wave_unit<__VA_ARGS__, -1, LIN_>(ap, l, xtab, qst, fnd, unit);        \
+        else if (x) wave_unit<__VA_ARGS__, 1, LIN_>(ap, l, xtab, qst, fnd, unit);          \
+        else wave_unit<__VA_ARGS__, 0, LIN_>(ap, l, xtab, qst, fnd, unit);                 \
+    } while (0)
+#if XH_RSUM_SINGLE_NXR
+#define XH_SINGLE(...)                                                                     \
+    do {                                                                                   \
+        if (lin) XH_BY_OUTLETS(true, __VA_ARGS__, 1);                                      \
+        else XH_BY_OUTLETS(false, __VA_ARGS__, 1);                                         \
+    } while (0)
+#else
+#define XH_SINGLE(...)                                                                     \
+    do {                                                                                   \
+        if (lin) wave_unit<__VA_ARGS__, 1, -1, true>(ap, l, xtab, qst, fnd, unit);         \
+        else wave_unit<__VA_ARGS__, 1, -1, false>(ap, l, xtab, qst, fnd, unit);            \
+    } while (0)
+#endif
+#define XH_NO_OUTLET(...)                                                                  \
+    do {                                                                                   \
+        if (lin) wave_unit<__VA_ARGS__, true>(ap, l, xtab, qst, fnd, unit);                \
+        else wave_unit<__VA_ARGS__, false>(ap, l, xtab, qst, fnd, unit);                   \
     } while (0)
     if (p & 16) {
-        if (!(p & 8) || (p & 4)) bad = true;
-        else if (g2) XH_BY_OUTLETS(1, 0, 2, true, true, false, 2);
-        else if (g) XH_BY_OUTLETS(1, 0, 1, true, true, false, 2);
-        else XH_BY_OUTLETS(1, 0, 0, true, true, false, 2);
-#undef XH_BY_OUTLETS
+        if (!(p & 8) || (p & 4) || (p & 32)) bad = true;
+        else if (g2) XH_BY_OUTLETS(false, 1, 0, 2, true, true, false, 2);
+        else if (g) XH_BY_OUTLETS(false, 1, 0, 1, true, true, false, 2);
+        else XH_BY_OUTLETS(false, 1, 0, 0, true, true, false, 2);
     } else if (p & 8) {
+        const bool lin = (p & 32) != 0 && A(linear) != 0;
         if (p & 4) {
             if (g || !A(fold_cell)) bad = true;
-            else wave_unit<1, 0, 0, true, true, true, 1>(ap, l, xtab, qst, fnd, unit);
-        } else if (g2) wave_unit<1, 0, 2, true, true, false, 1>(ap, l, xtab, qst, fnd, unit);
-        else if (g) wave_unit<1, 0, 1, true, true, false, 1>(ap, l, xtab, qst, fnd, unit);
-        else if ((p & 2) || x) wave_unit<1, 0, 0, true, true, false, 1>(ap, l, xtab, qst, fnd, unit);
-        else if (p & 1) wave_unit<1, 0, 0, false, true, false, 1>(ap, l, xtab, qst, fnd, unit);
-        else wave_unit<0, 0, 0, false, true, false, 1>(ap, l, xtab, qst, fnd, unit);
+            else XH_SINGLE(1, 0, 0, true, true, true);
+        } else if (g2) XH_SINGLE(1, 0, 2, true, true, false);
+        else if (g) XH_SINGLE(1, 0, 1, true, true, false);
+        else if ((p & 2) || x) XH_SINGLE(1, 0, 0, true, true, false);
+        else if (p & 1) XH_NO_OUTLET(1, 0, 0, false, true, false, 1, 0);
+        else XH_NO_OUTLET(0, 0, 0, false, true, false, 1, 0);
+#undef XH_NO_OUTLET
+#undef XH_SINGLE
+#undef XH_BY_OUTLETS
+    } else if (p & 32) {
+        bad = true;
     } else if (p & 4) {
         if (g || !A(fold_cell)) bad = true;
         else wave_unit<1, 0, 0, true, true, true>(ap, l, xtab, qst, fnd, unit);
diff --git a/xanthos_amd/csrc/xh_mrtm_wave_launch.hip b/xanthos_amd/csrc/xh_mrtm_wave_launch.hip
--- a/xanthos_amd/csrc/xh_mrtm_wave_launch.hip
+++ b/xanthos_amd/csrc/xh_mrtm_wave_launch.hip
@@ -172,6 +172,7 @@
         }
     }
     a.fold_cell = static_cast<const int *>(fp->d_fold_cell.p);
+    a.linear = xh_env_on("XH_RSUM_LINEAR", true) ? 1 : 0;
     if (!fp->d_skew_args) XH_HIP(ctx, hipMalloc(&fp->d_skew_args, sizeof(WaveArgs) + 256));
     hipLaunchKernelGGL(k_mrtm_wave_args, dim3(1), dim3(256), 0, st, a, static_cast<WaveArgs *>(fp->d_skew_args),
                        reinterpret_cast<uint4 *>(cnt), (unsigned)(x_cnt / sizeof(uint4)));
diff --git a/xanthos_amd/csrc/xh_mrtm_wave_unit.h b/xanthos_amd/csrc/xh_mrtm_wave_unit.h
--- a/xanthos_amd/csrc/xh_mrtm_wave_unit.h
+++ b/xanthos_amd/csrc/xh_mrtm_wave_unit.h
@@ -65,6 +65,7 @@
     unsigned *fault;
     unsigned long long *stats;
     const int *fold_cell;
+    int linear;
 };
 
 __device__ __forceinline__ unsigned ld_relaxed(const unsigned *p) {
@@ -123,7 +124,7 @@
     static __device__ __forceinline__ T zero() { return 0.0; }
 };
 
-template <int PRE, int POST, int NG, bool CHAIN, bool RSUM = false, bool FOLD = false, int SGL = 0, int NXR = -1>
+template <int PRE, int POST, int NG, bool CHAIN, bool RSUM = false, bool FOLD = false, int SGL = 0, int NXR = -1, bool LIN = false>
 __device__ __forceinline__ void wave_unit(WaveArgsK *ap, char *lds_generic, uint2 *xtab,
                                           __attribute__((address_space(3))) unsigned *qstage,
                                           __attribute__((address_space(3))) double *fend, const int unit) {
@@ -151,6 +152,7 @@
     static_assert(!RSUM || (PRE <= 1 && POST == 0), "reassociated form: one inflow entry");
     static_assert(!FOLD || (RSUM && NG == 0), "folded leaves: reassociated form, units without imports");
     static_assert(SGL == 0 || RSUM, "single-sum plans: reassociated form");
+    static_assert(!LIN || SGL == 1, "linear units: single units of a single-sum plan");
     const int gcL = FOLD ? A(fold_cell)[slot] : -1;
     const bool validL = FOLD && valid && gcL >= 0;
     const unsigned row_offL = (unsigned)(validL ? gcL : 0) * A(q_row_stride);
@@ -166,6 +168,7 @@
     unsigned gsgl = 0;
     bool xlane = false;
     double fmin_seen = 0.0;
+    double smin_seen = 0.0, Sp = 0.0;
     if (SGL != 0) {
         const unsigned lf = A(lane_flags)[slot];
         xlane = valid && (lf & 2u) != 0;
@@ -336,17 +339,19 @@
     const unsigned long long cyc_begin = __builtin_amdgcn_s_memtime();
     const unsigned long long rt_begin = __builtin_amdgcn_s_memrealtime();
 
-    unsigned seen_ready = 0, seen_done = 0, pend_ready = 0, pend_done = 0;
-    auto load_async = [&](const unsigned *q) {
-        unsigned v;
-        asm volatile("global_load_dword %0, %1, off sc1" : "=v"(v) : "v"(q) : "memory");
-        return v;
-    };
+    unsigned seen_ready = 0, seen_done = 0;
     auto check = [&](int n) {
         const unsigned long long w0 = __builtin_amdgcn_s_memtime();
-        asm volatile("s_waitcnt vmcnt(8)" : "+v"(pend_ready), "+v"(pend_done) : : "memory");
-        asm volatile("s_waitcnt vmcnt(0)" ::: "memory");
+        unsigned now_ready = 0, now_done = 0;
+        if (any_x || any_g)
+            asm volatile("global_load_dword %0, %2, off sc1\n\tglobal_load_dword %1, %3, off sc1\n\ts_waitcnt vmcnt(0)"
+                         : "=&v"(now_done), "=&v"(now_ready)
+                         : "v"(done_p), "v"(ready_p)
+                         : "memory");
+        else
+            asm volatile("s_waitcnt vmcnt(0)" ::: "memory");
         if (SGL == 2) gsgl |= (xlane && fmin_seen < -SGL_XEPS) ? 4u : 0u;
+        if (LIN) gsgl |= (smin_seen < -SGL_EPS) ? 8u : 0u;
         if ((FOLD && __any(gfold != 0)) || (SGL != 0 && __any(gsgl != 0))) {
             __hip_atomic_store(A(fault), FAULT_GUARD, __ATOMIC_RELAXED, __HIP_MEMORY_SCOPE_AGENT);
             alive = false;
@@ -357,7 +362,7 @@
             if (fenced) __builtin_amdgcn_fence(__ATOMIC_RELEASE, "agent");
             if (has_x) __hip_atomic_store(A(ready) + xedge, (unsigned)pub, __ATOMIC_RELAXED, __HIP_MEMORY_SCOPE_AGENT);
             const int need = n + CH - lmax - A(rs);
-            seen_done = max(seen_done, pend_done);
+            seen_done = max(seen_done, now_done);
             if (need > 0 && alive)
                 alive = wave_wait_ge(has_x, done_p, (unsigned)min(need, total), seen_done, A(fault), FAULT_RING_WAIT);
         }
@@ -367,13 +372,11 @@
                 __hip_atomic_store(A(done) + unit, (unsigned)min(max(n - glmax, 0), total), __ATOMIC_RELAXED,
                                    __HIP_MEMORY_SCOPE_AGENT);
             const int need = min(total, n + CH + GROUP - lag_g);
-            seen_ready = max(seen_ready, pend_ready);
+            seen_ready = max(seen_ready, now_ready);
             alive = wave_wait_ge(has_g && need > 0, ready_p, (unsigned)max(need, 0), seen_ready, A(fault), FAULT_DATA_WAIT);
             if (fenced) __builtin_amdgcn_fence(__ATOMIC_ACQUIRE, "agent");
             asm volatile("" ::: "memory");
         }
-        if (any_x) pend_done = load_async(done_p);
-        if (any_g) pend_ready = load_async(ready_p);
         cyc_wait_ring += w1 - w0;
         cyc_wait_data += __builtin_amdgcn_s_memtime() - w1;
     };
@@ -401,7 +404,8 @@
                 ob_a[j] = ob_a[j + 1];
             }
             ob_s[OB - 1] = snapS;
-            if constexpr (RSUM) ob_a[OB - 1] = snapA * f.inv_nt_prev;
+            if constexpr (LIN) ob_a[OB - 1] = (snapA * tauinv) * f.inv_nt_prev;
+            else if constexpr (RSUM) ob_a[OB - 1] = snapA * f.inv_nt_prev;
             else ob_a[OB - 1] = snapA / (double)f.nt_prev;
             if (FOLD) {
 #pragma unroll
@@ -554,7 +558,7 @@
                 if (edge == 1) S = c ? S0v : S;
                 if (FOLD && edge == 1) SL = c ? S0L : SL;
                 if (edge == 2) {
-                    if (c) fend[lane] = F;
+                    if (c) fend[lane] = LIN ? Sp * tauinv : F;
                     if (FOLD && c) fend[LANES + lane] = FL;
                 }
             }
@@ -582,7 +586,13 @@
                 favgL += FL;
                 base = __builtin_fma(FL, dt, base);
             }
-            if constexpr (SGL == 1) {
+            if constexpr (LIN) {
+                own[(j & (RING - 1)) * NSLOT] = CHAIN ? __builtin_fma(S, tauinv, rc) : F0;
+                favg += S;
+                Sp = S;
+                S = PRE ? __builtin_fma(ac[0], dt, base) : base;
+                smin_seen = __builtin_fmin(smin_seen, S);
+            } else if constexpr (SGL == 1) {
                 const double S1 = PRE ? __builtin_fma(ac[0], dt, base) : base;
                 const double m = __builtin_fmin(S1, 0.0);
                 const double f2 = __builtin_fma(m, dtinv, F0);
@@ -691,6 +701,7 @@
     }
     if (alive) {
         if (SGL == 2) gsgl |= (xlane && fmin_seen < -SGL_XEPS) ? 4u : 0u;
+        if (LIN) gsgl |= (smin_seen < -SGL_EPS) ? 8u : 0u;
         if ((FOLD && __any(gfold != 0)) || (SGL != 0 && __any(gsgl != 0))) {
             __hip_atomic_store(A(fault), FAULT_GUARD, __ATOMIC_RELAXED, __HIP_MEMORY_SCOPE_AGENT);
             alive = false;
@@ -726,8 +737,12 @@
         const unsigned hw = __builtin_amdgcn_s_getreg((4) | (0 << 6) | (31 << 11));
         const unsigned xcc = __builtin_amdgcn_s_getreg((20) | (0 << 6) | (3 << 11));
         st[3] = (unsigned long long)((PRE + POST + (CHAIN ? 1 : 0) + 1) & 15) | (any_g ? 16u : 0u) | (any_x ? 32u : 0u) |
-                (V8 ? 64u : 0u) | (guard_set ? 128u : 0u) | ((unsigned long long)hw << 8) | ((unsigned long long)(xcc & 15u) << 40) |
+                (V8 ? 64u : 0u) | (guard_set ? 128u : 0u) | ((unsigned long long)(hw & 0xffffu) << 8) | ((unsigned long long)(xcc & 15u) << 40) |
                 (zone_groups << 44);
+#ifndef XH_WAVE_PROFILE
+        st[3] |= ((unsigned long long)ng << 24) | ((unsigned long long)nx_out << 29) | (LIN ? 1ull << 34 : 0ull) |
+                 (NXR >= 0 ? 1ull << 35 : 0ull) | (1ull << 63);
+#endif
         st[4] = cyc_wait_data;
         st[5] = cyc_wait_ring;
 #ifdef XH_WAVE_PROFILE
```

Result: faster. 3.410 billion, median of 6 (+4.8%).
